# dronefreak/CABiNet

Hardware: AMD Instinct MI355X
Metric: 1024x1024 images/sec fwd+bwd (CABiNet-MobileNetV3-Large) (higher is better)
Workload: dtype f32; 1 GPU; BASELINE configs[2]: CABiNet-MobileNetV3-Large, 8x3x1024x1024 synthetic 8-class per GPU, fwd + 2x OhemCE + bwd + grad all-reduce + SGD step, HIP CAB/FFM kernels, fp32, random-init (model seed 0, gamma=0.5); per_gpu_batch=8, global_batch=8, n_classes=8, parallelism=dp1, miopen_find_mode=FAST

## Files before the change

cabinet_amd/_lib.py:

```python

from __future__ import annotations

import ctypes
import os
import threading

_PKG_DIR = os.path.dirname(os.path.abspath(__file__))
LIB_PATH = os.path.join(_PKG_DIR, "libcabinet_hip.so")
ABI_VERSION = 8

_c_float_p = ctypes.c_void_p
_INT, _FLT, _SZ, _PTR = ctypes.c_int, ctypes.c_float, ctypes.c_size_t, ctypes.c_void_p

SIGNATURES = {
    "cabinet_abi_version": (_INT, []),
    "cabinet_last_error": (ctypes.c_char_p, []),
    "cabinet_cab_attn_supported": (_INT, [_INT] * 2),
    "cabinet_cab_attn_precision_supported": (_INT, [_INT] * 3),
    "cabinet_cab_attn_fwd_workspace_bytes": (_SZ, [_INT] * 5),
    "cabinet_cab_attn_fwd": (_INT, [_PTR, _PTR, _PTR, _FLT, _INT, _INT, _INT, _INT, _INT, _PTR, _PTR, _PTR, _SZ, _PTR]),
    "cabinet_cab_attn_proj_supported": (_INT, [_INT] * 5),
    "cabinet_cab_attn_proj_fwd": (_INT, [_PTR] * 4 + [_FLT] + [_INT] * 5 + [_PTR] * 3 + [_PTR]),
    "cabinet_cab_attn_bwd_workspace_bytes": (_SZ, [_INT] * 4),
    "cabinet_cab_attn_bwd": (_INT, [_PTR] * 6 + [_FLT] + [_INT] * 4 + [_PTR] * 3 + [_PTR, _SZ, _PTR]),
    "cabinet_ffm_fwd_workspace_bytes": (_SZ, [_INT] * 7),
    "cabinet_ffm_fwd": (_INT, [_PTR] * 9 + [_INT] * 7 + [_INT, _FLT, _FLT] + [_PTR] * 6 + [_PTR, _SZ, _PTR]),
    "cabinet_ffm_bwd_workspace_bytes": (_SZ, [_INT] * 7),
    "cabinet_ffm_bwd": (_INT, [_PTR] * 13 + [_INT] * 7 + [_INT] + [_PTR] * 7 + [_PTR, _SZ, _PTR]),
    "cabinet_ffm_up_fwd_workspace_bytes": (_SZ, [_INT] * 9),
    "cabinet_ffm_up_fwd": (_INT, [_PTR] * 9 + [_INT] * 9 + [_INT, _FLT, _FLT, _INT] + [_PTR] * 6 + [_PTR, _SZ, _PTR]),
    "cabinet_ffm_up_bwd_workspace_bytes": (_SZ, [_INT] * 9),
    "cabinet_ffm_up_bwd": (_INT, [_PTR] * 13 + [_INT] * 9 + [_INT] + [_PTR] * 7 + [_PTR, _SZ, _PTR]),
    "cabinet_ohem_up_blocks": (_INT, [_INT] * 3),
    "cabinet_ohem_stats": (_INT, [_PTR, _PTR, _INT, _INT, _PTR, _PTR]),
    "cabinet_ohem_up_fwd": (_INT, [_PTR, _PTR] + [_INT] * 6 + [_FLT, _INT] + [_PTR] * 3 + [_PTR]),
    "cabinet_ohem_up_bwd_workspace_bytes": (_SZ, [_INT] * 6),
    "cabinet_ohem_up_bwd": (_INT, [_PTR] * 3 + [_INT] * 6 + [_FLT, _INT, _FLT] + [_PTR] + [_PTR, _SZ, _PTR]),
    "cabinet_ohem_up_pair_fwd": (_INT, [_PTR] * 3 + [_INT] * 6 + [_FLT, _INT] + [_PTR] * 3 + [_PTR]),
    "cabinet_ohem_up_pair_bwd_workspace_bytes": (_SZ, [_INT] * 6),
    "cabinet_ohem_up_pair_bwd": (_INT, [_PTR] * 4 + [_INT] * 6 + [_FLT, _INT, _FLT] + [_PTR] + [_PTR, _SZ, _PTR]),
    "cabinet_ohem_up_w_fwd": (_INT, [_PTR, _PTR] + [_INT] * 6 + [_FLT, _INT] + [_PTR] * 3 + [_PTR, _PTR]),
    "cabinet_ohem_up_w_bwd": (_INT, [_PTR] * 3 + [_INT] * 6 + [_FLT, _INT, _FLT] + [_PTR] + [_PTR, _SZ] + [_PTR, _PTR]),
    "cabinet_ohem_up_pair_w_fwd": (_INT, [_PTR] * 3 + [_INT] * 6 + [_FLT, _INT] + [_PTR] * 3 + [_PTR, _PTR, _PTR]),
    "cabinet_ohem_up_pair_w_bwd": (_INT, [_PTR] * 4 + [_INT] * 6 + [_FLT, _INT, _FLT] + [_PTR] + [_PTR, _SZ] + [_PTR, _PTR, _PTR]),
    "cabinet_ohem_select_workspace_bytes": (_SZ, [_INT] * 4),
    "cabinet_ohem_select": (_INT, [_PTR] * 3 + [_INT] * 5 + [_FLT] + [_INT] * 3 + [_PTR] * 3 + [_PTR, _SZ, _PTR]),
    "cabinet_ohem_up_w_bwd_sel": (_INT, [_PTR] * 3 + [_INT] * 6 + [_PTR, _INT, _FLT] + [_PTR] + [_PTR, _SZ] + [_PTR, _PTR]),
    "cabinet_ohem_up_pair_w_bwd_sel": (_INT, [_PTR] * 4 + [_INT] * 6 + [_PTR, _INT, _FLT] + [_PTR] + [_PTR, _SZ] + [_PTR, _PTR, _PTR]),
    "cabinet_cab_qkv_supported": (_INT, [_INT] * 7 + [_PTR]),
    "cabinet_cab_qkv_padded_bins": (_INT, [_INT, _PTR]),
    "cabinet_cab_qkv_fwd_workspace_bytes": (_SZ, [_INT] * 7 + [_PTR]),
    "cabinet_cab_qkv_fwd": (_INT, [_PTR] * 14 + [_INT] * 7 + [_PTR] + [_INT, _FLT, _FLT] + [_PTR] * 10
                            + [_PTR, _SZ, _PTR]),
    "cabinet_cab_qkv_bwd_workspace_bytes": (_SZ, [_INT] * 7 + [_PTR]),
    "cabinet_cab_qkv_bwd": (_INT, [_PTR] * 20 + [_INT] * 7 + [_PTR] + [_INT] + [_PTR] * 9 + [_PTR, _SZ, _PTR]),
    "cabinet_conv1x1_fwd_workspace_bytes": (_SZ, [_INT] * 2),
    "cabinet_conv1x1_fwd": (_INT, [_PTR] * 2 + [_INT] * 4 + [_PTR] + [_PTR, _SZ, _PTR]),
    "cabinet_conv1x1_bias_supported": (_INT, [_INT] * 4),
    "cabinet_conv1x1_bias_fwd": (_INT, [_PTR] * 3 + [_INT] * 4 + [_PTR] + [_PTR, _SZ, _PTR]),
    "cabinet_channel_sum": (_INT, [_PTR] + [_INT] * 3 + [_PTR] + [_PTR]),
    "cabinet_conv1x1_bwd_workspace_bytes": (_SZ, [_INT] * 4),
    "cabinet_conv1x1_bwd": (_INT, [_PTR] * 3 + [_INT] * 4 + [_PTR] * 2 + [_PTR, _SZ, _PTR]),
    "cabinet_bn_act_workspace_bytes": (_SZ, [_INT] * 3),
    "cabinet_bn_act_fwd": (_INT, [_PTR] * 6 + [_INT] * 5 + [_FLT, _FLT] + [_PTR] * 3 + [_PTR, _SZ, _PTR]),
    "cabinet_bn_act_bwd": (_INT, [_PTR] * 6 + [_INT] * 5 + [_PTR] * 3 + [_PTR, _SZ, _PTR]),
    "cabinet_bn_cls_supported": (_INT, [_INT] * 3),
    "cabinet_bn_cls_table_floats": (_INT, [_INT] * 2),
    "cabinet_bn_cls_fwd_workspace_bytes": (_SZ, [_INT] * 3),
    "cabinet_bn_cls_fwd": (_INT, [_PTR] * 8 + [_INT] * 6 + [_FLT, _FLT] + [_PTR] * 2 + [_PTR, _SZ, _PTR]),
    "cabinet_bn_cls_bwd_workspace_bytes": (_SZ, [_INT] * 4),
    "cabinet_bn_cls_bwd": (_INT, [_PTR] * 3 + [_INT] * 6 + [_PTR] * 5 + [_PTR, _SZ, _PTR]),
    "cabinet_gate_act_fwd": (_INT, [_PTR] * 2 + [_INT] * 4 + [_PTR] + [_PTR]),
    "cabinet_gate_act_bwd_workspace_bytes": (_SZ, [_INT] * 3),
    "cabinet_gate_act_bwd": (_INT, [_PTR] * 3 + [_INT] * 4 + [_PTR] * 2 + [_PTR, _SZ, _PTR]),
    "cabinet_bn_dwconv_fwd_workspace_bytes": (_SZ, [_INT] * 4),
    "cabinet_bn_dwconv_fwd": (_INT, [_PTR] * 6 + [_INT] * 8 + [_FLT, _FLT] + [_PTR] * 3 + [_PTR, _SZ, _PTR]),
    "cabinet_bn_dwconv_bwd_workspace_bytes": (_SZ, [_INT] * 6),
    "cabinet_bn_dwconv_bwd": (_INT, [_PTR] * 7 + [_INT] * 8 + [_PTR] * 4 + [_PTR, _SZ, _PTR]),
    "cabinet_stem_conv_fwd": (_INT, [_PTR] * 2 + [_INT] * 3 + [_PTR] + [_PTR]),
    "cabinet_stem_conv_wrw_workspace_bytes": (_SZ, [_INT] * 3),
    "cabinet_stem_conv_wrw": (_INT, [_PTR] * 2 + [_INT] * 3 + [_PTR] + [_PTR, _SZ, _PTR]),
    "cabinet_pwconv_supported": (_INT, [_INT] * 3),
    "cabinet_pwconv_fwd": (_INT, [_PTR] * 2 + [_INT] * 4 + [_PTR] + [_PTR]),
    "cabinet_pwconv_bwd_workspace_bytes": (_SZ, [_INT] * 4),
    "cabinet_pwconv_bwd": (_INT, [_PTR] * 3 + [_INT] * 4 + [_PTR] * 2 + [_PTR, _SZ, _PTR]),
    "cabinet_pwconv_wide_supported": (_INT, [_INT] * 3),
    "cabinet_pwconv_wide_wgrad_workspace_bytes": (_SZ, [_INT] * 4),
    "cabinet_pwconv_wide_wgrad": (_INT, [_PTR] * 2 + [_INT] * 4 + [_PTR] + [_PTR, _SZ, _PTR]),
    "cabinet_conv3x3s2_supported": (_INT, [_INT] * 2),
    "cabinet_conv3x3s2_wgrad_workspace_bytes": (_SZ, [_INT] * 5),
    "cabinet_conv3x3s2_wgrad": (_INT, [_PTR] * 2 + [_INT] * 5 + [_PTR] + [_PTR, _SZ, _PTR]),
    "cabinet_conv3x3s2_dgrad": (_INT, [_PTR] * 2 + [_INT] * 5 + [_PTR] + [_PTR]),
    "cabinet_bn_act_fwd_part": (_INT, [_PTR] * 7 + [_INT] * 6 + [_FLT, _FLT] + [_PTR] * 3 + [_PTR]),
    "cabinet_conv3x3_supported": (_INT, [_INT] * 3),
    "cabinet_conv3x3_tile_blocks": (_INT, [_INT] * 3),
    "cabinet_conv3x3_fwd_workspace_bytes": (_SZ, [_INT] * 6),
    "cabinet_conv3x3_fwd": (_INT, [_PTR] * 3 + [_INT] * 6 + [_PTR] * 2 + [_PTR, _SZ, _PTR]),
    "cabinet_conv3x3_bwd_workspace_bytes": (_SZ, [_INT] * 6),
    "cabinet_conv3x3_bwd": (_INT, [_PTR] * 4 + [_INT] * 6 + [_PTR] * 3 + [_PTR, _SZ, _PTR]),
    "cabinet_dwconv_supported": (_INT, [_INT] * 2),
    "cabinet_dwconv_fwd": (_INT, [_PTR] * 2 + [_INT] * 6 + [_PTR] + [_PTR]),
    "cabinet_dwconv_bwd_workspace_bytes": (_SZ, [_INT] * 6),
    "cabinet_dwconv_bwd": (_INT, [_PTR] * 3 + [_INT] * 6 + [_PTR] * 2 + [_PTR, _SZ, _PTR]),
    "cabinet_cab_local_supported": (_INT, [_INT] * 4),
    "cabinet_cab_local_fwd_workspace_bytes": (_SZ, [_INT] * 4),
    "cabinet_cab_local_bwd_workspace_bytes": (_SZ, [_INT] * 4),
    "cabinet_cab_local_fwd": (_INT, [_PTR] * 3 + [_PTR] * 5 + [_INT] * 5 + [_FLT, _FLT] + [_PTR] * 3 + [_PTR, _SZ, _PTR]),
    "cabinet_cab_local_bwd": (_INT, [_PTR] * 4 + [_PTR] * 3 + [_PTR] * 2 + [_INT] * 5 + [_PTR] * 3 + [_PTR] * 3 + [_PTR, _SZ, _PTR]),
    "cabinet_eval_chip_accum_supported": (_INT, [_INT] * 6),
    "cabinet_eval_chip_accum": (_INT, [_PTR] * 2 + [_INT] * 6 + [_PTR] + [_INT] * 4 + [_PTR] * 2 + [_PTR]),
    "cabinet_eval_scale_merge": (_INT, [_PTR] + [_INT] * 8 + [_PTR] + [_INT] * 2 + [_PTR]),
    "cabinet_eval_argmax_hist": (_INT, [_PTR] * 2 + [_INT] * 5 + [_PTR] * 2 + [_PTR]),
    "cabinet_se_act_bwd_workspace_bytes": (_SZ, [_INT] * 3),
    "cabinet_se_act_bwd_reduce": (_INT, [_PTR] * 8 + [_INT] * 4 + [_PTR] * 2 + [_PTR, _SZ, _PTR]),
    "cabinet_se_act_bwd_coef": (_INT, [_PTR] * 3 + [_INT] * 4 + [_PTR] * 4 + [_PTR]),
    "cabinet_se_act_bwd_dx": (_INT, [_PTR] * 9 + [_INT] * 4 + [_PTR] + [_PTR]),
}

_lock = threading.Lock()
_lib = None


def _preload_hip_runtime():
    import sys

    cands = []
    if "torch" in sys.modules:
        cands.append(os.path.join(os.path.dirname(sys.modules["torch"].__file__), "lib", "libamdhip64.so"))
    cands += ["libamdhip64.so.7", "/opt/rocm/lib/libamdhip64.so.7"]
    for c in cands:
        try:
            ctypes.CDLL(c, mode=ctypes.RTLD_GLOBAL)
            return c
        except OSError:
            continue
    raise RuntimeError("cabinet_amd: no HIP runtime (libamdhip64.so.7) could be loaded")


def load():
    global _lib
    if _lib is not None:
        return _lib
    with _lock:
        if _lib is not None:
            return _lib
        if not os.path.exists(LIB_PATH):
            raise RuntimeError(
                f"cabinet_amd: {LIB_PATH} is missing -- build it with `python -m cabinet_amd.build` "
                "(there is no non-HIP fallback for device tensors)")
        _preload_hip_runtime()
        lib = ctypes.CDLL(LIB_PATH)
        for name, (res, args) in SIGNATURES.items():
            try:
                fn = getattr(lib, name)
            except AttributeError as e:
                raise RuntimeError(f"cabinet_amd: {LIB_PATH} does not export {name}") from e
            fn.restype, fn.argtypes = res, args
        got = lib.cabinet_abi_version()
        if got != ABI_VERSION:
            raise RuntimeError(f"cabinet_amd: ABI version {got} != expected {ABI_VERSION}; rebuild the library")
        _lib = lib
    return _lib


def available() -> bool:
    return os.path.exists(LIB_PATH)


def check(rc: int, what: str):
    if rc != 0:
        msg = load().cabinet_last_error().decode("utf-8", "replace")
        raise RuntimeError(f"cabinet_amd: {what} failed (code {rc}): {msg}")
```

cabinet_amd/build.py:

```python

from __future__ import annotations

import argparse
import hashlib
import os
import shutil
import subprocess
import sys
from concurrent.futures import ThreadPoolExecutor

PKG_DIR = os.path.dirname(os.path.abspath(__file__))
CSRC = os.path.join(PKG_DIR, "csrc")
OBJ_DIR = os.path.join(PKG_DIR, "csrc", "build")
LIB_PATH = os.path.join(PKG_DIR, "libcabinet_hip.so")
ARCH = "gfx950"

SOURCES = ["capi.hip", "cab_attn_fwd.hip", "cab_attn_bf16.hip", "cab_attn_bwd.hip", "ffm.hip", "ffm_bwd_fused.hip", "ffm_bwd_adj.hip", "ffm_fwd_fused.hip", "gemm_bf16.hip", "ohem.hip", "cab_local.hip", "cab_local_tiled.hip", "cab_qkv.hip", "cab_qkv_fused.hip", "bn_act.hip", "dwconv.hip", "stem_conv.hip", "pwconv.hip", "pwconv_wide.hip", "conv3x3_s2.hip", "small_gemm.hip", "conv3x3_wino.hip", "bn_cls.hip", "eval_tail.hip"]
HEADERS = ["common.hpp", "cab_local.hpp", "cab_qkv.hpp", "blocks.hpp", "act.hpp", "bn_finalize.hpp", "slab_sum.hpp", os.path.join("..", "..", "include", "cabinet_hip.h")]


def _hipcc():
    for cand in (os.environ.get("HIPCC"), shutil.which("hipcc"), "/opt/rocm/bin/hipcc"):
        if cand and os.path.exists(cand):
            return cand
    raise RuntimeError("hipcc not found: cannot build libcabinet_hip.so")


def _digest(paths):
    h = hashlib.sha256()
    for p in paths:
        with open(p, "rb") as f:
            h.update(f.read())
    return h.hexdigest()


def source_digest():
    paths = [os.path.join(CSRC, s) for s in SOURCES] + [os.path.normpath(os.path.join(CSRC, h)) for h in HEADERS]
    return _digest(paths)


def is_fresh():
    stamp = LIB_PATH + ".stamp"
    if not (os.path.exists(LIB_PATH) and os.path.exists(stamp)):
        return False
    with open(stamp) as f:
        return f.read().strip() == _stamp()


def _stamp():
    return (source_digest() + " " + os.environ.get("CABINET_EXTRA_HIPCC_FLAGS", "").strip()).strip()


def build(force=False, save_temps=False, verbose=True):
    if not force and is_fresh():
        if verbose:
            print(f"[cabinet_amd.build] up to date: {LIB_PATH}")
        return LIB_PATH
    hipcc = _hipcc()
    os.makedirs(OBJ_DIR, exist_ok=True)
    flags = [f"--offload-arch={ARCH}", "-O3", "-fPIC", "-std=c++17", "-ffp-contract=off",
             "-Wall", "-Wno-unused-function"]
    if save_temps:
        flags.append("-save-temps=obj")
    flags += os.environ.get("CABINET_EXTRA_HIPCC_FLAGS", "").split()

    def compile_one(src):
        obj = os.path.join(OBJ_DIR, src.replace(".hip", ".o"))
        cmd = [hipcc, *flags, "-c", os.path.join(CSRC, src), "-o", obj]
        r = subprocess.run(cmd, capture_output=True, text=True)
        if r.returncode != 0:
            raise RuntimeError(f"hipcc failed for {src}:\n{r.stdout}\n{r.stderr}")
        if verbose and r.stderr.strip():
            print(r.stderr, file=sys.stderr)
        return obj

    with ThreadPoolExecutor(max_workers=min(len(SOURCES), os.cpu_count() or 4)) as ex:
        objs = list(ex.map(compile_one, SOURCES))
    link = [hipcc, f"--offload-arch={ARCH}", "-shared", "-fPIC", *objs, "-o", LIB_PATH,
            "-fno-rtlib-add-rpath", "-Wl,-soname,libcabinet_hip.so", "--hip-link"]
    r = subprocess.run(link, capture_output=True, text=True)
    if r.returncode != 0:
        raise RuntimeError(f"link failed:\n{r.stdout}\n{r.stderr}")
    with open(LIB_PATH + ".stamp", "w") as f:
        f.write(_stamp())
    if verbose:
        print(f"[cabinet_amd.build] built {LIB_PATH}")
    return LIB_PATH


if __name__ == "__main__":
    ap = argparse.ArgumentParser()
    ap.add_argument("--force", action="store_true")
    ap.add_argument("--save-temps", action="store_true")
    a = ap.parse_args()
    build(force=a.force, save_temps=a.save_temps)
```

cabinet_amd/csrc/act.hpp:

```cpp
#pragma once
#include <hip/hip_runtime.h>

namespace cabinet {

enum { ACT_NONE = 0, ACT_RELU = 1, ACT_HSWISH = 2 };

__device__ __forceinline__ float div6(float x) {
    const float c = 1.f / 6.f;
    const float q = x * c;
    return fmaf(fmaf(-6.f, q, x), c, q);
}

__device__ __forceinline__ float act_fwd(float u, int act) {
    if (act == ACT_RELU) return fmaxf(u, 0.f);
    if (act == ACT_HSWISH) return div6(u * fminf(fmaxf(u + 3.f, 0.f), 6.f));
    return u;
}
__device__ __forceinline__ float act_grad(float u, int act) {
    if (act == ACT_RELU) return u > 0.f ? 1.f : 0.f;
    if (act == ACT_HSWISH) {
        const float t = u + 3.f;
        const float inner = (t > 0.f && t < 6.f) ? div6(u) : 0.f;
        return div6(fminf(fmaxf(t, 0.f), 6.f)) + inner;
    }
    return 1.f;
}

struct BnFold {
    const float *mean, *invstd, *weight, *bias;
    int act;
};

size_t bn_act_workspace(int B, int C, int P);
hipError_t bn_stats_run(const float* x, float* running_mean, float* running_var, int B, int C, int P, int training,
                        float momentum, float eps, float* save_mean, float* save_invstd, void* ws, hipStream_t stream);
hipError_t bn_bwd_tail_run(const float* part, int nt, const float* dy, const float* x, const float* weight,
                           const float* bias, const float* save_mean, const float* save_invstd, int B, int C, int P,
                           int act, int training, float* dx, float* dweight, float* dbias, float* coef,
                           hipStream_t stream);

}
```

cabinet_amd/csrc/bn_act.hip:

```cpp
#include "act.hpp"
#include "bn_finalize.hpp"
#include "common.hpp"

namespace cabinet {


__device__ __forceinline__ int ba_load(const float* __restrict__ row, int P, int lo, f32x4 (&v)[BA_V]) {
    const int hi = min(lo + BA_CHUNK, P);
    if ((P & 3) == 0) {
#pragma unroll
        for (int i = 0; i < BA_V; ++i) {
            const int p = lo + (i * BA_T + threadIdx.x) * 4;
            v[i] = p < hi ? *reinterpret_cast<const f32x4*>(row + p) : f32x4{0.f, 0.f, 0.f, 0.f};
        }
    } else {
#pragma unroll
        for (int i = 0; i < BA_V; ++i)
#pragma unroll
            for (int e = 0; e < 4; ++e) {
                const int p = lo + (i * BA_T + threadIdx.x) * 4 + e;
                v[i][e] = p < hi ? row[p] : 0.f;
            }
    }
    return hi - lo;
// ... 215 lines not shown
    f32x4 vz[BA_V], vg[BA_V];
    ba_load(z + (size_t)row * P, P, ch * BA_CHUNK, vz);
    ba_load(dy + (size_t)row * P, P, ch * BA_CHUNK, vg);
    float s1 = 0.f, s2 = 0.f, s3 = 0.f;
#pragma unroll
    for (int i = 0; i < BA_V; ++i)
#pragma unroll
        for (int e = 0; e < 4; ++e) {
            const float xh = (vz[i][e] - mu) * inv;
            const float du = vg[i][e] * act_grad(fmaf(xh, gam, bet) * gt, act);
            s1 += du, s2 = fmaf(du, xh, s2);
            if (ba_valid(P, ch * BA_CHUNK, i, e)) s3 += xh;
        }
    s1 = block_sum_256(s1, red);
    s2 = block_sum_256(s2, red);
    s3 = block_sum_256(s3, red);
    if (threadIdx.x == 0) {
        part[(size_t)row * chunks + ch] = s1;
        part[((size_t)rows + row) * chunks + ch] = s2;
        part[((size_t)2 * rows + row) * chunks + ch] = s3;
    }
}

__global__ void se_bwd_gate_kernel(const float* __restrict__ part, int rows, int C, int chunks, const float* __restrict__ weight,
                                   const float* __restrict__ bias, const float* __restrict__ a2, float* __restrict__ sums,
                                   float* __restrict__ da2) {
    const int row = blockIdx.x * blockDim.x + threadIdx.x;
    if (row >= rows) return;
    float s[3];
#pragma unroll
    for (int k = 0; k < 3; ++k) {
        float t = 0.f;
        for (int j = 0; j < chunks; ++j) t += part[((size_t)k * rows + row) * chunks + j];
        sums[(size_t)k * rows + row] = s[k] = t;
    }
    const int c = row % C;
    const float dgate = weight[c] * s[1] + bias[c] * s[0], u = a2[row] + 3.f;
    da2[row] = (u > 0.f && u < 6.f) ? dgate / 6.f : 0.f;
}

__global__ void se_bwd_coef_kernel(const float* __restrict__ sums, const float* __restrict__ gate, const float* __restrict__ ds,
                                   int B, int C, int P, int training, float* __restrict__ dweight, float* __restrict__ dbias,
                                   float* __restrict__ coef, float* __restrict__ ds_p) {
    const int c = blockIdx.x * blockDim.x + threadIdx.x;
    if (c >= C) return;
    const int rows = B * C;
    float db = 0.f, dw = 0.f;
    for (int b = 0; b < B; ++b) {
        const int row = b * C + c;
        const float g = gate[row], d = ds[row], dp = d / (float)P;
        ds_p[row] = dp;
        db += g * sums[row] + d;
        dw += g * sums[rows + row] + dp * sums[2 * rows + row];
    }
    dbias[c] = db;
    dweight[c] = dw;
    const float n = (float)B * (float)P;
    coef[c] = training ? db / n : 0.f;
    coef[C + c] = training ? dw / n : 0.f;
}

__global__ __launch_bounds__(BA_T) void se_bwd_dx_kernel(const float* __restrict__ dy, const float* __restrict__ z,
                                                         const float* __restrict__ mean, const float* __restrict__ invstd,
                                                         const float* __restrict__ weight, const float* __restrict__ bias,
                                                         const float* __restrict__ gate, const float* __restrict__ ds_p,
                                                         const float* __restrict__ coef, int C, int P, int chunks, int act,
                                                         float* __restrict__ dz) {
    const int row = blockIdx.x / chunks, ch = blockIdx.x - row * chunks, c = row % C;
    const float mu = mean[c], inv = invstd[c], gam = weight[c], bet = bias[c], gt = gate[row], dp = ds_p[row];
    const float m1 = coef[c], m2 = coef[C + c], gi = gam * inv;
    f32x4 vz[BA_V], vg[BA_V];
    ba_load(z + (size_t)row * P, P, ch * BA_CHUNK, vz);
    ba_load(dy + (size_t)row * P, P, ch * BA_CHUNK, vg);
#pragma unroll
    for (int i = 0; i < BA_V; ++i)
#pragma unroll
        for (int e = 0; e < 4; ++e) {
            const float xh = (vz[i][e] - mu) * inv;
            const float du = vg[i][e] * act_grad(fmaf(xh, gam, bet) * gt, act);
            vg[i][e] = gi * (fmaf(gt, du, dp) - m1 - xh * m2);
        }
    ba_store(dz + (size_t)row * P, P, ch * BA_CHUNK, vg);
}

static int ba_chunks(int P) { return ceil_div(P, BA_CHUNK); }

size_t se_act_bwd_workspace(int B, int C, int P) { return align_up((size_t)3 * B * C * ba_chunks(P) * sizeof(float), 256); }

hipError_t se_act_bwd_reduce_run(const float* dy, const float* z, const float* mean, const float* invstd, const float* weight,
                                 const float* bias, const float* gate, const float* a2, int B, int C, int P, int act, float* sums,
                                 float* da2, void* ws, hipStream_t stream) {
    const int chunks = ba_chunks(P), rows = B * C;
    float* part = static_cast<float*>(ws);
    hipLaunchKernelGGL(se_bwd_reduce_kernel, dim3(rows * chunks), dim3(BA_T), 0, stream, dy, z, mean, invstd, weight, bias, gate,
                       rows, C, P, chunks, act, part);
    hipLaunchKernelGGL(se_bwd_gate_kernel, dim3(ceil_div(rows, 256)), dim3(256), 0, stream, part, rows, C, chunks, weight, bias, a2,
                       sums, da2);
    return hipGetLastError();
}

hipError_t se_act_bwd_coef_run(const float* sums, const float* gate, const float* ds, int B, int C, int P, int training,
                               float* dweight, float* dbias, float* coef, float* ds_p, hipStream_t stream) {
    hipLaunchKernelGGL(se_bwd_coef_kernel, dim3(ceil_div(C, 256)), dim3(256), 0, stream, sums, gate, ds, B, C, P, training, dweight,
                       dbias, coef, ds_p);
    return hipGetLastError();
}

hipError_t se_act_bwd_dx_run(const float* dy, const float* z, const float* mean, const float* invstd, const float* weight,
                             const float* bias, const float* gate, const float* ds_p, const float* coef, int B, int C, int P,
                             int act, float* dz, hipStream_t stream) {
    const int chunks = ba_chunks(P);
    hipLaunchKernelGGL(se_bwd_dx_kernel, dim3(B * C * chunks), dim3(BA_T), 0, stream, dy, z, mean, invstd, weight, bias, gate,
                       ds_p, coef, C, P, chunks, act, dz);
    return hipGetLastError();
}

size_t bn_act_workspace(int B, int C, int P) {
    return align_up((size_t)2 * C * B * ba_chunks(P) * sizeof(float), 256) + align_up((size_t)2 * C * sizeof(float), 256);
}

hipError_t bn_stats_run(const float* x, float* running_mean, float* running_var, int B, int C, int P, int training,
                        float momentum, float eps, float* save_mean, float* save_invstd, void* ws, hipStream_t stream) {
    const int chunks = ba_chunks(P), grid = B * C * chunks;
    float* part = static_cast<float*>(ws);
    if (training)
        hipLaunchKernelGGL(bn_act_stats_kernel, dim3(grid), dim3(BA_T), 0, stream, x, part, B, C, P, chunks);
    hipLaunchKernelGGL(bn_act_finalize_kernel, dim3(C), dim3(BA_T), 0, stream, part, B, C, P, chunks, 0, 0, training, momentum,
                       eps, running_mean, running_var, save_mean, save_invstd);
    return hipGetLastError();
}

hipError_t bn_act_fwd_part_run(const float* x, const float* conv_part, int H, int W, const float* weight, const float* bias,
                               float* running_mean, float* running_var, const float* residual, int B, int C, int act, int training,
                               float momentum, float eps, float* y, float* save_mean, float* save_invstd, hipStream_t stream) {
    const int P = H * W, chunks = ba_chunks(P), grid = B * C * chunks;
    hipLaunchKernelGGL(bn_act_finalize_kernel, dim3(C), dim3(BA_T), 0, stream, conv_part, B, C, P, chunks, H, W, training, momentum,
                       eps, running_mean, running_var, save_mean, save_invstd);
    hipLaunchKernelGGL(bn_act_apply_kernel, dim3(grid), dim3(BA_T), 0, stream, x, save_mean, save_invstd, weight, bias,
                       residual, C, P, chunks, act, y);
    return hipGetLastError();
}

hipError_t bn_act_fwd_run(const float* x, const float* weight, const float* bias, float* running_mean,
                          float* running_var, const float* residual, int B, int C, int P, int act, int training,
                          float momentum, float eps, float* y, float* save_mean, float* save_invstd, void* ws,
                          hipStream_t stream) {
    const int chunks = ba_chunks(P), grid = B * C * chunks;
    (void)bn_stats_run(x, running_mean, running_var, B, C, P, training, momentum, eps, save_mean, save_invstd, ws, stream);
    hipLaunchKernelGGL(bn_act_apply_kernel, dim3(grid), dim3(BA_T), 0, stream, x, save_mean, save_invstd, weight, bias,
                       residual, C, P, chunks, act, y);
    return hipGetLastError();
}

hipError_t bn_bwd_tail_run(const float* part, int nt, const float* dy, const float* x, const float* weight,
                           const float* bias, const float* save_mean, const float* save_invstd, int B, int C, int P,
                           int act, int training, float* dx, float* dweight, float* dbias, float* coef,
                           hipStream_t stream) {
    const int chunks = ba_chunks(P), grid = B * C * chunks;
    hipLaunchKernelGGL(bn_act_bwd_finalize_kernel, dim3(C), dim3(BA_T), 0, stream, part, nt, C, (double)B * (double)P,
                       training, dweight, dbias, coef);
    hipLaunchKernelGGL(bn_act_bwd_dx_kernel, dim3(grid), dim3(BA_T), 0, stream, dy, x, save_mean, save_invstd, weight,
                       bias, coef, C, P, chunks, act, dx);
    return hipGetLastError();
}

hipError_t bn_act_bwd_run(const float* dy, const float* x, const float* weight, const float* bias,
                          const float* save_mean, const float* save_invstd, int B, int C, int P, int act, int training,
                          float* dx, float* dweight, float* dbias, void* ws, hipStream_t stream) {
    const int chunks = ba_chunks(P), grid = B * C * chunks, nt = B * chunks;
    float* part = static_cast<float*>(ws);
    float* coef = reinterpret_cast<float*>(static_cast<char*>(ws) + align_up((size_t)2 * C * nt * sizeof(float), 256));
    hipLaunchKernelGGL(bn_act_bwd_reduce_kernel, dim3(grid), dim3(BA_T), 0, stream, dy, x, save_mean, save_invstd, weight,
                       bias, B, C, P, chunks, act, part);
    return bn_bwd_tail_run(part, nt, dy, x, weight, bias, save_mean, save_invstd, B, C, P, act, training, dx, dweight,
                           dbias, coef, stream);
}

size_t gate_act_workspace(int rows, int P) { return align_up((size_t)rows * ba_chunks(P) * sizeof(float), 256); }

hipError_t gate_act_fwd_run(const float* x, const float* gate, int rows, int P, int act, float* y, hipStream_t stream) {
    const int chunks = ba_chunks(P);
    hipLaunchKernelGGL(gate_act_fwd_kernel, dim3(rows * chunks), dim3(BA_T), 0, stream, x, gate, P, chunks, act, y);
    return hipGetLastError();
}

hipError_t gate_act_bwd_run(const float* dy, const float* x, const float* gate, int rows, int P, int act, float* dx,
                            float* dgate, void* ws, hipStream_t stream) {
    const int chunks = ba_chunks(P);
    float* part = static_cast<float*>(ws);
    hipLaunchKernelGGL(gate_act_bwd_kernel, dim3(rows * chunks), dim3(BA_T), 0, stream, dy, x, gate, P, chunks, act, dx,
                       part);
    hipLaunchKernelGGL(gate_act_dgate_kernel, dim3(ceil_div(rows, 256)), dim3(256), 0, stream, part, rows, chunks, dgate);
    return hipGetLastError();
}

}
```

cabinet_amd/csrc/capi.hip:

```cpp
#include "../../include/cabinet_hip.h"

#include <stdarg.h>
#include <stdint.h>
#include <stdio.h>

#include "blocks.hpp"
#include "cab_local.hpp"
#include "cab_qkv.hpp"
#include "common.hpp"

namespace cabinet {
int attn_fwd_kvsplit(int B, int n);
bool attn_shape_supported(int Kc, int Vc);
hipError_t attn_fwd_dispatch(const float* q, const float* k, const float* v, float scale, int B, int Kc,
                             int Vc, int n, float* ctx, float* lse, float* part_ctx, float* part_lse,
                             int kvsplit, hipStream_t stream);
bool attn_fwd_proj_supported(int B, int Kc, int Vc, int Co, int n);
hipError_t attn_fwd_proj_dispatch(const float* q, const float* k, const float* v, const float* w_out, float scale, int B, int Kc,
                                  int Vc, int Co, int n, float* ctx, float* glob, float* lse, hipStream_t stream);
bool attn_bf16_supported(int Kc, int Vc);
size_t attn_bf16_pack_bytes(int B, int Kc, int Vc, int n, int precision);
hipError_t attn_fwd_bf16_dispatch(const float* q, const float* k, const float* v, float scale, int B, int Kc, int Vc, int n,
                                  float* ctx, float* lse, float* part_ctx, float* part_lse, int kvsplit, void* pack, int precision,
                                  hipStream_t stream);
size_t attn_bwd_workspace(int B, int Kc, int Vc, int n);
hipError_t attn_bwd_dispatch(const float* dctx, const float* q, const float* k, const float* v,
                             const float* ctx, const float* lse, float scale, int B, int Kc, int Vc, int n,
                             float* dq, float* dk, float* dv, void* ws, hipStream_t stream);
struct FfmShape {
    int B, Cs, Cc, Co, Cm, H, W;
};
size_t ffm_fwd_workspace(const FfmShape& s);
size_t ffm_bwd_workspace(const FfmShape& s);
hipError_t ffm_fwd_run(const FfmShape& s, const float* fsp, const float* fcp, const float* w_blk,
                       const float* bn_w, const float* bn_b, float* run_mean, float* run_var,
                       const float* w1, const float* w2, int training, float momentum, float eps, float* out,
                       float* z, float* save_mean, float* save_invstd, float* pooled, float* gate, void* ws,
                       hipStream_t stream);
size_t ffm_up_fwd_workspace(const FfmShape& s, int Hl, int Wl);
size_t ffm_up_bwd_workspace(const FfmShape& s, int Hl, int Wl);
hipError_t ffm_up_fwd_run(const FfmShape& s, int Hl, int Wl, const float* fsp, const float* low,
                          const float* w_blk, const float* bn_w, const float* bn_b, float* run_mean,
                          float* run_var, const float* w1, const float* w2, int training, float momentum,
                          float eps, float* out, float* z, float* save_mean, float* save_invstd, float* pooled,
                          float* gate, void* ws, int precision, hipStream_t stream);
hipError_t ffm_up_bwd_run(const FfmShape& s, int Hl, int Wl, const float* dout, const float* fsp,
                          const float* low, const float* w_blk, const float* bn_w, const float* bn_b,
                          const float* w1, const float* w2, const float* z, const float* save_mean,
                          const float* save_invstd, const float* pooled, const float* gate, int training,
                          float* dfsp, float* dlow, float* dw_blk, float* dbn_w, float* dbn_b, float* dw1,
                          float* dw2, void* ws, hipStream_t stream);
hipError_t ffm_bwd_run(const FfmShape& s, const float* dout, const float* fsp, const float* fcp,
                       const float* w_blk, const float* bn_w, const float* bn_b, const float* w1,
                       const float* w2, const float* z, const float* save_mean, const float* save_invstd,
                       const float* pooled, const float* gate, int training, float* dfsp, float* dfcp,
                       float* dw_blk, float* dbn_w, float* dbn_b, float* dw1, float* dw2, void* ws,
                       hipStream_t stream);
size_t bn_act_workspace(int B, int C, int P);
hipError_t bn_act_fwd_run(const float* x, const float* weight, const float* bias, float* running_mean,
                          float* running_var, const float* residual, int B, int C, int P, int act, int training,
                          float momentum, float eps, float* y, float* save_mean, float* save_invstd, void* ws,
                          hipStream_t stream);
hipError_t bn_act_bwd_run(const float* dy, const float* x, const float* weight, const float* bias,
                          const float* save_mean, const float* save_invstd, int B, int C, int P, int act, int training,
                          float* dx, float* dweight, float* dbias, void* ws, hipStream_t stream);
hipError_t bn_act_fwd_part_run(const float* x, const float* conv_part, int H, int W, const float* weight, const float* bias,
                               float* running_mean, float* running_var, const float* residual, int B, int C, int act, int training,
                               float momentum, float eps, float* y, float* save_mean, float* save_invstd, hipStream_t stream);
size_t se_act_bwd_workspace(int B, int C, int P);
hipError_t se_act_bwd_reduce_run(const float* dy, const float* z, const float* mean, const float* invstd, const float* weight,
                                 const float* bias, const float* gate, const float* a2, int B, int C, int P, int act, float* sums,
                                 float* da2, void* ws, hipStream_t stream);
hipError_t se_act_bwd_coef_run(const float* sums, const float* gate, const float* ds, int B, int C, int P, int training,
                               float* dweight, float* dbias, float* coef, float* ds_p, hipStream_t stream);
hipError_t se_act_bwd_dx_run(const float* dy, const float* z, const float* mean, const float* invstd, const float* weight,
                             const float* bias, const float* gate, const float* ds_p, const float* coef, int B, int C, int P,
                             int act, float* dz, hipStream_t stream);
size_t gate_act_workspace(int rows, int P);
hipError_t gate_act_fwd_run(const float* x, const float* gate, int rows, int P, int act, float* y, hipStream_t stream);
hipError_t gate_act_bwd_run(const float* dy, const float* x, const float* gate, int rows, int P, int act, float* dx,
                            float* dgate, void* ws, hipStream_t stream);
bool bn_cls_supported(int C, int K, int P);
int bn_cls_table_floats(int C, int K);
size_t bn_cls_fwd_workspace(int B, int C, int P);
size_t bn_cls_bwd_workspace(int B, int C, int K, int P);
hipError_t bn_cls_fwd_run(const float* z, const float* conv_part, const float* bn_w, const float* bn_b, float* run_mean, float* run_var,
                          const float* w_cls, const float* bias, int B, int C, int K, int H, int W, int training, float momentum,
                          float eps, float* y, float* tab, void* ws, hipStream_t stream);
hipError_t bn_cls_bwd_run(const float* dy, const float* z, const float* tab, int B, int C, int K, int H, int W, int training, float* dz,
                          float* dbn_w, float* dbn_b, float* dw_cls, float* dbias, void* ws, hipStream_t stream);
bool dwconv_supported(int K, int S);
size_t dwconv_bwd_workspace(int B, int C, int H, int W, int K);
hipError_t dwconv_fwd_run(const float* x, const float* w, int B, int C, int H, int W, int K, int S, float* y,
                          hipStream_t stream);
hipError_t dwconv_bwd_run(const float* dy, const float* x, const float* w, int B, int C, int H, int W, int K, int S,
                          float* dx, float* dw, void* ws, hipStream_t stream);
size_t bn_dwconv_fwd_workspace(int B, int C, int H, int W);
size_t bn_dwconv_bwd_workspace(int B, int C, int H, int W, int K);
hipError_t bn_dwconv_fwd_run(const float* z, const float* bn_w, const float* bn_b, float* run_mean, float* run_var,
                             const float* w, int B, int C, int H, int W, int K, int S, int act, int training,
                             float momentum, float eps, float* y, float* save_mean, float* save_invstd, void* ws,
                             hipStream_t stream);
hipError_t bn_dwconv_bwd_run(const float* dy, const float* z, const float* bn_w, const float* bn_b,
                             const float* save_mean, const float* save_invstd, const float* w, int B, int C, int H,
                             int W, int K, int S, int act, int training, float* dz, float* dbn_w, float* dbn_b,
                             float* dw, void* ws, hipStream_t stream);
size_t stem_conv_wrw_workspace(int B, int H, int W);
hipError_t stem_conv_fwd_run(const float* x, const float* w, int B, int H, int W, float* y, hipStream_t stream);
hipError_t stem_conv_wrw_run(const float* dy, const float* x, int B, int H, int W, float* dw, void* ws,
                             hipStream_t stream);
bool pwconv_wide_supported(int Ci, int Co, int P);
size_t pwconv_wide_wgrad_workspace(int B, int Ci, int Co, int P);
hipError_t pwconv_wide_wgrad_run(const float* dy, const float* x, int B, int Ci, int Co, int P, float* dw, void* ws,
                                 hipStream_t stream);
bool conv3x3s2_supported(int Ci, int Co);
long long conv3x3s2_wgrad_slabs(int B, int Ci, int H, int W);
size_t conv3x3s2_wgrad_workspace(int B, int Ci, int H, int W);
hipError_t conv3x3s2_wgrad_run(const float* dy, const float* x, int B, int Ci, int H, int W, float* dw, void* ws,
                               hipStream_t stream);
long long conv3x3s2_dgrad_workgroups(int B, int H, int W);
hipError_t conv3x3s2_dgrad_run(const float* dy, const float* w, int B, int H, int W, float* dx, hipStream_t stream);
bool pwconv_supported(int Ci, int Co, int P);
size_t pwconv_bwd_workspace(int B, int Ci, int Co, int P);
hipError_t pwconv_fwd_run(const float* x, const float* w, int B, int Ci, int Co, int P, float* y, hipStream_t stream);
hipError_t pwconv_bwd_run(const float* dy, const float* x, const float* w, int B, int Ci, int Co, int P, float* dx,
                          float* dw, void* ws, hipStream_t stream);
int ohem_blocks(int B, int H, int W);
hipError_t ohem_up_fwd_run(int nh, const float* const* low, const long long* labels, int B, int C, int Hl, int Wl, int H, int W,
                           float thresh, int ignore_lb, float* const* loss_px, float* const* blk_sum, int* const* blk_cnt,
                           const float* const* class_weight, hipStream_t stream);
hipError_t ohem_stats_run(const float* blk_sum, const int* blk_cnt, int nheads, int nblk, double* stats, hipStream_t stream);
size_t ohem_up_bwd_workspace(int B, int C, int H, int Wl);
bool ohem_up_supported(int C, int Wl, int W);
hipError_t ohem_up_bwd_run(int nh, const float* const* low, const long long* labels, const float* const* loss_px, int B, int C,
                           int Hl, int Wl, int H, int W, float thresh, int ignore_lb, float coef, float* dlow, void* ws,
                           const float* const* cw, const double* dsel, hipStream_t stream);
size_t ohem_select_workspace(int nheads);
hipError_t ohem_select_run(int nheads, const float* const* loss_px, const long long* labels, const double* stats, long long P, int C,
                           float thresh, const int* n_min, int ignore_lb, const float* const* cw, double* sel, void* ws,
                           hipStream_t stream);
struct WinoShape {
    int B, C0, C1, K, H, W;
};
bool conv3x3_supported(int C0, int C1, int K);
bool conv3x3_shape_ok(const WinoShape& s);
int conv3x3_tile_blocks(int B, int H, int W);
size_t conv3x3_fwd_workspace(const WinoShape& s);
size_t conv3x3_bwd_workspace(const WinoShape& s);
hipError_t conv3x3_fwd_run(const WinoShape& s, const float* x0, const float* x1, const float* w, float* y, float* stat_part, void* ws,
                           hipStream_t stream);
hipError_t conv3x3_bwd_run(const WinoShape& s, const float* dy, const float* x0, const float* x1, const float* w, float* dx0,
                           float* dx1, float* dw, void* ws, hipStream_t stream);
int eval_chip_threads(int C, int wl, int cw, int nsrc);
hipError_t eval_chip_accum_run(const float* a, const float* b, int N, int C, int hl, int wl, int ch, int cw, float* dst, int FH,
                               int FW, int y0, int x0, const float* rcp_y, const float* rcp_x, hipStream_t stream);
hipError_t eval_scale_merge_run(const float* prob, int N, int C, int FH, int FW, int hst, int hed, int wst, int wed, float* total,
                                int H, int W, hipStream_t stream);
hipError_t eval_argmax_hist_run(const float* total, const long long* labels, int N, int C, int H, int W, int ignore_lb, long long* hist,
                                unsigned char* pred, hipStream_t stream);
}

static thread_local char g_err[512] = "";

static int fail(int code, const char* fmt, ...) {
    va_list ap;
    va_start(ap, fmt);
    vsnprintf(g_err, sizeof(g_err), fmt, ap);
    va_end(ap);
    return code;
}

template <typename... P>
static bool aligned16(P... p) {
    return ((reinterpret_cast<uintptr_t>(p) | ...) & 15) == 0;
}
#define CABINET_REQUIRE_ALIGNED(what, ...)                                                                            \
    if (!aligned16(__VA_ARGS__))                                                                                      \
    return fail(CABINET_ERR_INVALID_ARG, what ": tensor pointers must be 16-byte aligned (128-bit loads / stores)")

static int hip_status(hipError_t e, const char* what) {
    if (e == hipSuccess) return CABINET_OK;
    return fail(CABINET_ERR_HIP, "%s: %s", what, hipGetErrorString(e));
}

extern "C" {

int cabinet_abi_version(void) { return CABINET_ABI_VERSION; }
const char* cabinet_last_error(void) { return g_err; }

static int check_attn_shape(int B, int Kc, int Vc, int n) {
    if (B <= 0 || Kc <= 0 || Vc <= 0 || n <= 0)
        return fail(CABINET_ERR_INVALID_ARG, "cab_attn: non-positive dimension B=%d Kc=%d Vc=%d n=%d", B, Kc,
                    Vc, n);
    if (!cabinet::attn_shape_supported(Kc, Vc))
        return fail(CABINET_ERR_UNSUPPORTED,
                    "cab_attn: (Kc=%d, Vc=%d) has no gfx950 instantiation; built: (128,128) (256,128) (64,64)",
                    Kc, Vc);
    if (B > 65535) return fail(CABINET_ERR_UNSUPPORTED, "cab_attn: B=%d exceeds grid.z", B);
    return CABINET_OK;
}

int cabinet_cab_attn_supported(int Kc, int Vc) { return cabinet::attn_shape_supported(Kc, Vc) ? 1 : 0; }

int cabinet_cab_attn_precision_supported(int Kc, int Vc, int precision) {
    if (precision == CABINET_PREC_FP32) return cabinet_cab_attn_supported(Kc, Vc);
    if (precision == CABINET_PREC_BF16X3 || precision == CABINET_PREC_BF16X6) return cabinet::attn_bf16_supported(Kc, Vc) ? 1 : 0;
    return 0;
}

static size_t attn_fwd_split_bytes(int B, int Vc, int n, int split) {
    if (split == 1) return 0;
    return align_up((size_t)split * B * Vc * n * sizeof(float), 256) + align_up((size_t)split * B * n * sizeof(float), 256);
}

size_t cabinet_cab_attn_fwd_workspace_bytes(int B, int Kc, int Vc, int n, int precision) {
    if (B <= 0 || Kc <= 0 || Vc <= 0 || n <= 0 || !cabinet_cab_attn_precision_supported(Kc, Vc, precision)) return 0;
    const size_t pack = precision == CABINET_PREC_FP32 ? 0 : cabinet::attn_bf16_pack_bytes(B, Kc, Vc, n, precision);
    return attn_fwd_split_bytes(B, Vc, n, cabinet::attn_fwd_kvsplit(B, n)) + pack;
}

int cabinet_cab_attn_fwd(const float* q, const float* k, const float* v, float scale, int B, int Kc, int Vc,
                         int n, int precision, float* ctx, float* lse, void* workspace, size_t workspace_bytes,
                         cabinet_stream_t stream) {
    if (int rc = check_attn_shape(B, Kc, Vc, n)) return rc;
    if (!cabinet_cab_attn_precision_supported(Kc, Vc, precision))
        return fail(CABINET_ERR_UNSUPPORTED, "cab_attn_fwd: precision %d is not built for (Kc=%d, Vc=%d)", precision, Kc, Vc);
    if (!q || !k || !v || !ctx || !lse) return fail(CABINET_ERR_INVALID_ARG, "cab_attn_fwd: null tensor pointer");
    CABINET_REQUIRE_ALIGNED("cab_attn_fwd", q, k, v, ctx, lse);
    const size_t need = cabinet_cab_attn_fwd_workspace_bytes(B, Kc, Vc, n, precision);
    if (need && (!workspace || workspace_bytes < need))
        return fail(CABINET_ERR_WORKSPACE, "cab_attn_fwd: workspace %zu < %zu bytes", workspace_bytes, need);
    const int split = cabinet::attn_fwd_kvsplit(B, n);
    float* part_ctx = static_cast<float*>(workspace);
    float* part_lse = split > 1 ? reinterpret_cast<float*>(static_cast<char*>(workspace) +
                                                           align_up((size_t)split * B * Vc * n * sizeof(float), 256))
                                : nullptr;
    if (precision != CABINET_PREC_FP32) {
        void* pack = static_cast<char*>(workspace) + attn_fwd_split_bytes(B, Vc, n, split);
        return hip_status(cabinet::attn_fwd_bf16_dispatch(q, k, v, scale, B, Kc, Vc, n, ctx, lse, part_ctx, part_lse, split, pack,
                                                          precision, static_cast<hipStream_t>(stream)),
                          "cab_attn_fwd (split bf16) launch");
    }
    return hip_status(cabinet::attn_fwd_dispatch(q, k, v, scale, B, Kc, Vc, n, ctx, lse, part_ctx, part_lse,
                                                 split, static_cast<hipStream_t>(stream)),
                      "cab_attn_fwd launch");
}

int cabinet_cab_attn_proj_supported(int B, int Kc, int Vc, int Co, int n) {
    return cabinet::attn_fwd_proj_supported(B, Kc, Vc, Co, n) ? 1 : 0;
}

int cabinet_cab_attn_proj_fwd(const float* q, const float* k, const float* v, const float* w_out, float scale, int B, int Kc,
                              int Vc, int Co, int n, float* ctx, float* glob, float* lse, cabinet_stream_t stream) {
    if (int rc = check_attn_shape(B, Kc, Vc, n)) return rc;
    if (Co <= 0) return fail(CABINET_ERR_INVALID_ARG, "cab_attn_proj_fwd: non-positive Co=%d", Co);
    if (!cabinet::attn_fwd_proj_supported(B, Kc, Vc, Co, n))
        return fail(CABINET_ERR_UNSUPPORTED,
                    "cab_attn_proj_fwd: (B=%d, Kc=%d, Vc=%d, Co=%d, n=%d) is outside the fused form (see "
                    "cabinet_cab_attn_proj_supported); use cabinet_cab_attn_fwd + cabinet_conv1x1_fwd",
                    B, Kc, Vc, Co, n);
    if (!q || !k || !v || !w_out || !glob || !lse) return fail(CABINET_ERR_INVALID_ARG, "cab_attn_proj_fwd: null tensor pointer");
    CABINET_REQUIRE_ALIGNED("cab_attn_proj_fwd", q, k, v, w_out, ctx, glob, lse);
    return hip_status(cabinet::attn_fwd_proj_dispatch(q, k, v, w_out, scale, B, Kc, Vc, Co, n, ctx, glob, lse,
// ... 703 lines not shown
                       int stride, float* dx, float* dw, void* workspace, size_t workspace_bytes,
                       cabinet_stream_t stream) {
    if (int rc = check_dwconv(B, C, H, W, K, stride, "dwconv_bwd")) return rc;
    if (!dy || !x || !weight || !dx || !dw) return fail(CABINET_ERR_INVALID_ARG, "dwconv_bwd: null tensor pointer");
    const size_t need = cabinet::dwconv_bwd_workspace(B, C, H, W, K);
    if (!workspace || workspace_bytes < need)
        return fail(CABINET_ERR_WORKSPACE, "dwconv_bwd: workspace %zu < %zu bytes", workspace_bytes, need);
    return hip_status(cabinet::dwconv_bwd_run(dy, x, weight, B, C, H, W, K, stride, dx, dw, workspace,
                                              static_cast<hipStream_t>(stream)),
                      "dwconv_bwd launch");
}

int cabinet_gate_act_fwd(const float* x, const float* gate, int B, int C, int P, int act, float* y,
                         cabinet_stream_t stream) {
    if (int rc = check_bn_act(B, C, P, act, "gate_act_fwd")) return rc;
    if (!x || !gate || !y) return fail(CABINET_ERR_INVALID_ARG, "gate_act_fwd: null tensor pointer");
    return hip_status(cabinet::gate_act_fwd_run(x, gate, B * C, P, act, y, static_cast<hipStream_t>(stream)),
                      "gate_act_fwd launch");
}

size_t cabinet_gate_act_bwd_workspace_bytes(int B, int C, int P) {
    return B > 0 && C > 0 && P > 0 ? cabinet::gate_act_workspace(B * C, P) : 0;
}

int cabinet_gate_act_bwd(const float* dy, const float* x, const float* gate, int B, int C, int P, int act, float* dx,
                         float* dgate, void* workspace, size_t workspace_bytes, cabinet_stream_t stream) {
    if (int rc = check_bn_act(B, C, P, act, "gate_act_bwd")) return rc;
    if (!dy || !x || !gate || !dx || !dgate) return fail(CABINET_ERR_INVALID_ARG, "gate_act_bwd: null tensor pointer");
    const size_t need = cabinet::gate_act_workspace(B * C, P);
    if (!workspace || workspace_bytes < need)
        return fail(CABINET_ERR_WORKSPACE, "gate_act_bwd: workspace %zu < %zu bytes", workspace_bytes, need);
    return hip_status(cabinet::gate_act_bwd_run(dy, x, gate, B * C, P, act, dx, dgate, workspace,
                                                static_cast<hipStream_t>(stream)),
                      "gate_act_bwd launch");
}

size_t cabinet_se_act_bwd_workspace_bytes(int B, int C, int P) {
    return B > 0 && C > 0 && P > 0 ? cabinet::se_act_bwd_workspace(B, C, P) : 0;
}

int cabinet_se_act_bwd_reduce(const float* dy, const float* z, const float* mean, const float* invstd, const float* bn_weight,
                              const float* bn_bias, const float* gate, const float* a2, int B, int C, int P, int act, float* sums,
                              float* da2, void* workspace, size_t workspace_bytes, cabinet_stream_t stream) {
    if (int rc = check_bn_act(B, C, P, act, "se_act_bwd_reduce")) return rc;
    if (!dy || !z || !mean || !invstd || !bn_weight || !bn_bias || !gate || !a2 || !sums || !da2)
        return fail(CABINET_ERR_INVALID_ARG, "se_act_bwd_reduce: null tensor pointer");
    CABINET_REQUIRE_ALIGNED("se_act_bwd_reduce", dy, z);
    const size_t need = cabinet::se_act_bwd_workspace(B, C, P);
    if (!workspace || workspace_bytes < need)
        return fail(CABINET_ERR_WORKSPACE, "se_act_bwd_reduce: workspace %zu < %zu bytes", workspace_bytes, need);
    return hip_status(cabinet::se_act_bwd_reduce_run(dy, z, mean, invstd, bn_weight, bn_bias, gate, a2, B, C, P, act, sums, da2,
                                                     workspace, static_cast<hipStream_t>(stream)),
                      "se_act_bwd_reduce launch");
}

int cabinet_se_act_bwd_coef(const float* sums, const float* gate, const float* ds, int B, int C, int P, int training,
                            float* dbn_weight, float* dbn_bias, float* coef, float* ds_over_p, cabinet_stream_t stream) {
    if (B <= 0 || C <= 0 || P <= 0) return fail(CABINET_ERR_INVALID_ARG, "se_act_bwd_coef: non-positive dimension");
    if (!sums || !gate || !ds || !dbn_weight || !dbn_bias || !coef || !ds_over_p)
        return fail(CABINET_ERR_INVALID_ARG, "se_act_bwd_coef: null tensor pointer");
    return hip_status(cabinet::se_act_bwd_coef_run(sums, gate, ds, B, C, P, training, dbn_weight, dbn_bias, coef, ds_over_p,
                                                   static_cast<hipStream_t>(stream)),
                      "se_act_bwd_coef launch");
}

int cabinet_se_act_bwd_dx(const float* dy, const float* z, const float* mean, const float* invstd, const float* bn_weight,
                          const float* bn_bias, const float* gate, const float* ds_over_p, const float* coef, int B, int C, int P,
                          int act, float* dz, cabinet_stream_t stream) {
    if (int rc = check_bn_act(B, C, P, act, "se_act_bwd_dx")) return rc;
    if (!dy || !z || !mean || !invstd || !bn_weight || !bn_bias || !gate || !ds_over_p || !coef || !dz)
        return fail(CABINET_ERR_INVALID_ARG, "se_act_bwd_dx: null tensor pointer");
    CABINET_REQUIRE_ALIGNED("se_act_bwd_dx", dy, z, dz);
    return hip_status(cabinet::se_act_bwd_dx_run(dy, z, mean, invstd, bn_weight, bn_bias, gate, ds_over_p, coef, B, C, P, act, dz,
                                                 static_cast<hipStream_t>(stream)),
                      "se_act_bwd_dx launch");
}

size_t cabinet_bn_dwconv_fwd_workspace_bytes(int B, int C, int H, int W) {
    return B > 0 && C > 0 && H > 0 && W > 0 ? cabinet::bn_dwconv_fwd_workspace(B, C, H, W) : 0;
}

int cabinet_bn_dwconv_fwd(const float* z, const float* bn_weight, const float* bn_bias, float* running_mean,
                          float* running_var, const float* conv_weight, int B, int C, int H, int W, int K, int stride,
                          int act, int training, float momentum, float eps, float* y, float* save_mean,
                          float* save_invstd, void* workspace, size_t workspace_bytes, cabinet_stream_t stream) {
    if (int rc = check_dwconv(B, C, H, W, K, stride, "bn_dwconv_fwd")) return rc;
    if (int rc = check_bn_act(B, C, H * W, act, "bn_dwconv_fwd")) return rc;
    if (!z || !bn_weight || !bn_bias || !running_mean || !running_var || !conv_weight || !y || !save_mean || !save_invstd)
        return fail(CABINET_ERR_INVALID_ARG, "bn_dwconv_fwd: null tensor pointer");
    const size_t need = cabinet::bn_dwconv_fwd_workspace(B, C, H, W);
    if (!workspace || workspace_bytes < need)
        return fail(CABINET_ERR_WORKSPACE, "bn_dwconv_fwd: workspace %zu < %zu bytes", workspace_bytes, need);
    return hip_status(cabinet::bn_dwconv_fwd_run(z, bn_weight, bn_bias, running_mean, running_var, conv_weight, B, C, H, W,
                                                 K, stride, act, training, momentum, eps, y, save_mean, save_invstd,
                                                 workspace, static_cast<hipStream_t>(stream)),
                      "bn_dwconv_fwd launch");
}

size_t cabinet_bn_dwconv_bwd_workspace_bytes(int B, int C, int H, int W, int K, int stride) {
    if (B <= 0 || C <= 0 || H <= 0 || W <= 0 || !cabinet::dwconv_supported(K, stride)) return 0;
    return cabinet::bn_dwconv_bwd_workspace(B, C, H, W, K);
}

int cabinet_bn_dwconv_bwd(const float* dy, const float* z, const float* bn_weight, const float* bn_bias,
                          const float* save_mean, const float* save_invstd, const float* conv_weight, int B, int C,
                          int H, int W, int K, int stride, int act, int training, float* dz, float* dbn_weight,
                          float* dbn_bias, float* dconv_weight, void* workspace, size_t workspace_bytes,
                          cabinet_stream_t stream) {
    if (int rc = check_dwconv(B, C, H, W, K, stride, "bn_dwconv_bwd")) return rc;
    if (int rc = check_bn_act(B, C, H * W, act, "bn_dwconv_bwd")) return rc;
    if (!dy || !z || !bn_weight || !bn_bias || !save_mean || !save_invstd || !conv_weight || !dz || !dbn_weight ||
        !dbn_bias || !dconv_weight)
        return fail(CABINET_ERR_INVALID_ARG, "bn_dwconv_bwd: null tensor pointer");
    const size_t need = cabinet::bn_dwconv_bwd_workspace(B, C, H, W, K);
    if (!workspace || workspace_bytes < need)
        return fail(CABINET_ERR_WORKSPACE, "bn_dwconv_bwd: workspace %zu < %zu bytes", workspace_bytes, need);
    return hip_status(cabinet::bn_dwconv_bwd_run(dy, z, bn_weight, bn_bias, save_mean, save_invstd, conv_weight, B, C, H,
                                                 W, K, stride, act, training, dz, dbn_weight, dbn_bias, dconv_weight,
                                                 workspace, static_cast<hipStream_t>(stream)),
                      "bn_dwconv_bwd launch");
}

static int check_stem(int B, int H, int W, const char* who) {
    if (B <= 0 || H <= 0 || W <= 0) return fail(CABINET_ERR_INVALID_ARG, "%s: non-positive dimension", who);
    if ((long long)B * ((H + 1) / 2) > 2147483647LL / 4) return fail(CABINET_ERR_UNSUPPORTED, "%s: grid too large", who);
    return CABINET_OK;
}

int cabinet_stem_conv_fwd(const float* x, const float* weight, int B, int H, int W, float* y, cabinet_stream_t stream) {
    if (int rc = check_stem(B, H, W, "stem_conv_fwd")) return rc;
    if (!x || !weight || !y) return fail(CABINET_ERR_INVALID_ARG, "stem_conv_fwd: null tensor pointer");
    return hip_status(cabinet::stem_conv_fwd_run(x, weight, B, H, W, y, static_cast<hipStream_t>(stream)),
                      "stem_conv_fwd launch");
}

size_t cabinet_stem_conv_wrw_workspace_bytes(int B, int H, int W) {
    return B > 0 && H > 0 && W > 0 ? cabinet::stem_conv_wrw_workspace(B, H, W) : 0;
}

int cabinet_stem_conv_wrw(const float* dy, const float* x, int B, int H, int W, float* dw, void* workspace,
                          size_t workspace_bytes, cabinet_stream_t stream) {
    if (int rc = check_stem(B, H, W, "stem_conv_wrw")) return rc;
    if (!dy || !x || !dw) return fail(CABINET_ERR_INVALID_ARG, "stem_conv_wrw: null tensor pointer");
    const size_t need = cabinet::stem_conv_wrw_workspace(B, H, W);
    if (!workspace || workspace_bytes < need)
        return fail(CABINET_ERR_WORKSPACE, "stem_conv_wrw: workspace %zu < %zu bytes", workspace_bytes, need);
    return hip_status(cabinet::stem_conv_wrw_run(dy, x, B, H, W, dw, workspace, static_cast<hipStream_t>(stream)),
                      "stem_conv_wrw launch");
}

static int check_pwconv(int B, int Ci, int Co, int P, const char* who) {
    if (B <= 0 || Ci <= 0 || Co <= 0 || P <= 0) return fail(CABINET_ERR_INVALID_ARG, "%s: non-positive dimension", who);
    if (!cabinet::pwconv_supported(Ci, Co, P))
        return fail(CABINET_ERR_UNSUPPORTED, "%s: Ci=%d, Co=%d (multiples of 8, <= 120, block product <= 8)", who, Ci, Co);
    return CABINET_OK;
}

int cabinet_pwconv_supported(int Ci, int Co, int P) {
    return Ci > 0 && Co > 0 && P > 0 && cabinet::pwconv_supported(Ci, Co, P) ? 1 : 0;
}

int cabinet_pwconv_fwd(const float* x, const float* w, int B, int Ci, int Co, int P, float* y, cabinet_stream_t stream) {
    if (int rc = check_pwconv(B, Ci, Co, P, "pwconv_fwd")) return rc;
    if (!x || !w || !y) return fail(CABINET_ERR_INVALID_ARG, "pwconv_fwd: null tensor pointer");
    return hip_status(cabinet::pwconv_fwd_run(x, w, B, Ci, Co, P, y, static_cast<hipStream_t>(stream)),
                      "pwconv_fwd launch");
}

size_t cabinet_pwconv_bwd_workspace_bytes(int B, int Ci, int Co, int P) {
    if (B <= 0 || Ci <= 0 || Co <= 0 || P <= 0 || !cabinet::pwconv_supported(Ci, Co, P)) return 0;
    return cabinet::pwconv_bwd_workspace(B, Ci, Co, P);
}

int cabinet_pwconv_bwd(const float* dy, const float* x, const float* w, int B, int Ci, int Co, int P, float* dx,
                       float* dw, void* workspace, size_t workspace_bytes, cabinet_stream_t stream) {
    if (int rc = check_pwconv(B, Ci, Co, P, "pwconv_bwd")) return rc;
    if (!dy || !x || !w) return fail(CABINET_ERR_INVALID_ARG, "pwconv_bwd: null tensor pointer");
    const size_t need = cabinet::pwconv_bwd_workspace(B, Ci, Co, P);
    if (dw && (!workspace || workspace_bytes < need))
        return fail(CABINET_ERR_WORKSPACE, "pwconv_bwd: workspace %zu < %zu bytes", workspace_bytes, need);
    return hip_status(cabinet::pwconv_bwd_run(dy, x, w, B, Ci, Co, P, dx, dw, workspace, static_cast<hipStream_t>(stream)),
                      "pwconv_bwd launch");
}

int cabinet_pwconv_wide_supported(int Ci, int Co, int P) {
    return Ci > 0 && Co > 0 && P > 0 && cabinet::pwconv_wide_supported(Ci, Co, P) ? 1 : 0;
}

size_t cabinet_pwconv_wide_wgrad_workspace_bytes(int B, int Ci, int Co, int P) {
    if (B <= 0 || Ci <= 0 || Co <= 0 || P <= 0 || !cabinet::pwconv_wide_supported(Ci, Co, P)) return 0;
    if ((long long)B * ((P + 63) / 64) > (1ll << 30)) return 0;
    return cabinet::pwconv_wide_wgrad_workspace(B, Ci, Co, P);
}

int cabinet_pwconv_wide_wgrad(const float* dy, const float* x, int B, int Ci, int Co, int P, float* dw, void* workspace,
                              size_t workspace_bytes, cabinet_stream_t stream) {
    if (B <= 0 || Ci <= 0 || Co <= 0 || P <= 0)
        return fail(CABINET_ERR_INVALID_ARG, "pwconv_wide_wgrad: non-positive dimension");
    if ((long long)B * ((P + 63) / 64) > (1ll << 30))
        return fail(CABINET_ERR_UNSUPPORTED, "pwconv_wide_wgrad: B=%d, P=%d: more than 2^30 pixel chunks", B, P);
    if (!cabinet::pwconv_wide_supported(Ci, Co, P))
        return fail(CABINET_ERR_UNSUPPORTED, "pwconv_wide_wgrad: Ci=%d, Co=%d, P=%d (multiples of 8, <= 4096, P <= 2^21, max(Ci, Co) * P <= 2^28)",
                    Ci, Co, P);
    if (!dy || !x || !dw) return fail(CABINET_ERR_INVALID_ARG, "pwconv_wide_wgrad: null tensor pointer");
    const size_t need = cabinet::pwconv_wide_wgrad_workspace(B, Ci, Co, P);
    if (!workspace || workspace_bytes < need)
        return fail(CABINET_ERR_WORKSPACE, "pwconv_wide_wgrad: workspace %zu < %zu bytes", workspace_bytes, need);
    return hip_status(cabinet::pwconv_wide_wgrad_run(dy, x, B, Ci, Co, P, dw, workspace, static_cast<hipStream_t>(stream)),
                      "pwconv_wide_wgrad launch");
}

static bool conv3x3s2_size_ok(int B, int Ci, int H, int W) {
    return cabinet::conv3x3s2_wgrad_slabs(B, Ci, H, W) <= (1ll << 30);
}

int cabinet_conv3x3s2_supported(int Ci, int Co) { return cabinet::conv3x3s2_supported(Ci, Co) ? 1 : 0; }

size_t cabinet_conv3x3s2_wgrad_workspace_bytes(int B, int Ci, int Co, int H, int W) {
    if (B <= 0 || H <= 0 || W <= 0 || !cabinet::conv3x3s2_supported(Ci, Co) || !conv3x3s2_size_ok(B, Ci, H, W)) return 0;
    return cabinet::conv3x3s2_wgrad_workspace(B, Ci, H, W);
}

int cabinet_conv3x3s2_wgrad(const float* dy, const float* x, int B, int Ci, int Co, int H, int W, float* dw, void* workspace,
                            size_t workspace_bytes, cabinet_stream_t stream) {
    if (B <= 0 || Ci <= 0 || Co <= 0 || H <= 0 || W <= 0)
        return fail(CABINET_ERR_INVALID_ARG, "conv3x3s2_wgrad: non-positive dimension");
    if (!cabinet::conv3x3s2_supported(Ci, Co))
        return fail(CABINET_ERR_UNSUPPORTED, "conv3x3s2_wgrad: Ci=%d, Co=%d ((64, 64) and (3, 16) are compiled)", Ci, Co);
    if (!conv3x3s2_size_ok(B, Ci, H, W))
        return fail(CABINET_ERR_UNSUPPORTED, "conv3x3s2_wgrad: B=%d, H=%d, W=%d: grid too large", B, H, W);
    if (!dy || !x || !dw) return fail(CABINET_ERR_INVALID_ARG, "conv3x3s2_wgrad: null tensor pointer");
    const size_t need = cabinet::conv3x3s2_wgrad_workspace(B, Ci, H, W);
    if (!workspace || workspace_bytes < need)
        return fail(CABINET_ERR_WORKSPACE, "conv3x3s2_wgrad: workspace %zu < %zu bytes", workspace_bytes, need);
    return hip_status(cabinet::conv3x3s2_wgrad_run(dy, x, B, Ci, H, W, dw, workspace, static_cast<hipStream_t>(stream)),
                      "conv3x3s2_wgrad launch");
}

int cabinet_conv3x3s2_dgrad(const float* dy, const float* w, int B, int Ci, int Co, int H, int W, float* dx,
                            cabinet_stream_t stream) {
    if (B <= 0 || Ci <= 0 || Co <= 0 || H <= 0 || W <= 0)
        return fail(CABINET_ERR_INVALID_ARG, "conv3x3s2_dgrad: non-positive dimension");
    if (Ci != 64 || Co != 64)
        return fail(CABINET_ERR_UNSUPPORTED, "conv3x3s2_dgrad: Ci=%d, Co=%d ((64, 64) is compiled)", Ci, Co);
    if (cabinet::conv3x3s2_dgrad_workgroups(B, H, W) > (1ll << 30))
        return fail(CABINET_ERR_UNSUPPORTED, "conv3x3s2_dgrad: B=%d, H=%d, W=%d: grid too large", B, H, W);
    if (!dy || !w || !dx) return fail(CABINET_ERR_INVALID_ARG, "conv3x3s2_dgrad: null tensor pointer");
    if ((reinterpret_cast<size_t>(dx) & 7) != 0)
        return fail(CABINET_ERR_INVALID_ARG, "conv3x3s2_dgrad: dx must be 8-byte aligned");
    return hip_status(cabinet::conv3x3s2_dgrad_run(dy, w, B, H, W, dx, static_cast<hipStream_t>(stream)), "conv3x3s2_dgrad launch");
}

static int check_conv3x3(const cabinet::WinoShape& s, const char* who) {
    if (s.B <= 0 || s.C0 <= 0 || s.C1 < 0 || s.K <= 0 || s.H <= 0 || s.W <= 0)
        return fail(CABINET_ERR_INVALID_ARG, "%s: non-positive dimension", who);
    if (!cabinet::conv3x3_shape_ok(s))
        return fail(CABINET_ERR_UNSUPPORTED,
                    "%s: C0=%d C1=%d Co=%d H=%d W=%d (C0, C1 multiples of 16; Co, C0+C1 multiples of 64; C0 %% 64 == 0 when C1 > 0; "
                    "one image's tensors < 1 GiB)", who, s.C0, s.C1, s.K, s.H, s.W);
    return CABINET_OK;
}

int cabinet_conv3x3_supported(int C0, int C1, int Co) { return cabinet::conv3x3_supported(C0, C1, Co) ? 1 : 0; }

int cabinet_conv3x3_tile_blocks(int B, int H, int W) {
    return B > 0 && H > 0 && W > 0 ? cabinet::conv3x3_tile_blocks(B, H, W) : 0;
}

size_t cabinet_conv3x3_fwd_workspace_bytes(int B, int C0, int C1, int Co, int H, int W) {
    const cabinet::WinoShape s{B, C0, C1, Co, H, W};
    return B > 0 && H > 0 && W > 0 && cabinet::conv3x3_shape_ok(s) ? cabinet::conv3x3_fwd_workspace(s) : 0;
}

int cabinet_conv3x3_fwd(const float* x0, const float* x1, const float* w, int B, int C0, int C1, int Co, int H, int W, float* y,
                        float* bn_part, void* workspace, size_t workspace_bytes, cabinet_stream_t stream) {
    const cabinet::WinoShape s{B, C0, C1, Co, H, W};
    if (int rc = check_conv3x3(s, "conv3x3_fwd")) return rc;
    if (!x0 || !w || !y || (C1 > 0 && !x1)) return fail(CABINET_ERR_INVALID_ARG, "conv3x3_fwd: null tensor pointer");
    CABINET_REQUIRE_ALIGNED("conv3x3_fwd", x0, x1, w, y, bn_part);
    const size_t need = cabinet::conv3x3_fwd_workspace(s);
    if (!workspace || workspace_bytes < need)
        return fail(CABINET_ERR_WORKSPACE, "conv3x3_fwd: workspace %zu < %zu bytes", workspace_bytes, need);
    return hip_status(cabinet::conv3x3_fwd_run(s, x0, C1 > 0 ? x1 : nullptr, w, y, bn_part, workspace, static_cast<hipStream_t>(stream)),
                      "conv3x3_fwd launch");
}

size_t cabinet_conv3x3_bwd_workspace_bytes(int B, int C0, int C1, int Co, int H, int W) {
    const cabinet::WinoShape s{B, C0, C1, Co, H, W};
    return B > 0 && H > 0 && W > 0 && cabinet::conv3x3_shape_ok(s) ? cabinet::conv3x3_bwd_workspace(s) : 0;
}

int cabinet_conv3x3_bwd(const float* dy, const float* x0, const float* x1, const float* w, int B, int C0, int C1, int Co, int H,
                        int W, float* dx0, float* dx1, float* dw, void* workspace, size_t workspace_bytes, cabinet_stream_t stream) {
    const cabinet::WinoShape s{B, C0, C1, Co, H, W};
    if (int rc = check_conv3x3(s, "conv3x3_bwd")) return rc;
    if (!dy || !w || (dw && (!x0 || (C1 > 0 && !x1))) || (dx0 && C1 > 0 && !dx1))
        return fail(CABINET_ERR_INVALID_ARG, "conv3x3_bwd: null tensor pointer");
    CABINET_REQUIRE_ALIGNED("conv3x3_bwd", dy, x0, x1, w, dx0, dx1, dw);
    const size_t need = cabinet::conv3x3_bwd_workspace(s);
    if (!workspace || workspace_bytes < need)
        return fail(CABINET_ERR_WORKSPACE, "conv3x3_bwd: workspace %zu < %zu bytes", workspace_bytes, need);
    return hip_status(cabinet::conv3x3_bwd_run(s, dy, x0, C1 > 0 ? x1 : nullptr, w, dx0, C1 > 0 ? dx1 : nullptr, dw, workspace,
                                               static_cast<hipStream_t>(stream)),
                      "conv3x3_bwd launch");
}

int cabinet_eval_chip_accum_supported(int C, int hl, int wl, int ch, int cw, int flip) {
    if (C < 1 || C > 32 || hl < 1 || wl < 1 || ch < 1 || cw < 1 || ch > 65535) return 0;
    return cabinet::eval_chip_threads(C, wl, cw, flip ? 2 : 1) > 0 ? 1 : 0;
}

int cabinet_eval_chip_accum(const float* a, const float* b, int N, int C, int hl, int wl, int ch, int cw, float* dst, int FH, int FW,
                            int y0, int x0, const float* rcp_y, const float* rcp_x, cabinet_stream_t stream) {
    if (N <= 0 || C <= 0 || hl <= 0 || wl <= 0 || ch <= 0 || cw <= 0 || FH <= 0 || FW <= 0)
        return fail(CABINET_ERR_INVALID_ARG, "eval_chip_accum: non-positive dimension");
    if (!a || !dst) return fail(CABINET_ERR_INVALID_ARG, "eval_chip_accum: null tensor pointer");
    if (y0 < 0 || x0 < 0 || y0 > FH - ch || x0 > FW - cw)
        return fail(CABINET_ERR_INVALID_ARG, "eval_chip_accum: window (%d,%d)+(%d,%d) leaves the %dx%d destination", y0, x0, ch, cw, FH, FW);
    if (C > 32) return fail(CABINET_ERR_UNSUPPORTED, "eval_chip_accum: C=%d classes (max 32)", C);
    if (N > 65535 || ch > 65535) return fail(CABINET_ERR_UNSUPPORTED, "eval_chip_accum: N or chip height exceeds grid limits");
    if (!cabinet_eval_chip_accum_supported(C, hl, wl, ch, cw, b != nullptr))
        return fail(CABINET_ERR_UNSUPPORTED, "eval_chip_accum: C=%d x resize ratio %d/%d exceeds the LDS row buffers", C, wl, cw);
    return hip_status(cabinet::eval_chip_accum_run(a, b, N, C, hl, wl, ch, cw, dst, FH, FW, y0, x0, rcp_y, rcp_x,
                                                   static_cast<hipStream_t>(stream)),
                      "eval_chip_accum launch");
}

int cabinet_eval_scale_merge(const float* prob, int N, int C, int FH, int FW, int hst, int hed, int wst, int wed, float* total, int H,
                             int W, cabinet_stream_t stream) {
    if (N <= 0 || C <= 0 || FH <= 0 || FW <= 0 || H <= 0 || W <= 0)
        return fail(CABINET_ERR_INVALID_ARG, "eval_scale_merge: non-positive dimension");
    if (!prob || !total) return fail(CABINET_ERR_INVALID_ARG, "eval_scale_merge: null tensor pointer");
    if (hst < 0 || wst < 0 || hed <= hst || wed <= wst || hed > FH || wed > FW)
        return fail(CABINET_ERR_INVALID_ARG, "eval_scale_merge: crop [%d:%d, %d:%d] leaves the %dx%d source", hst, hed, wst, wed, FH, FW);
    if ((long long)N * C > 65535 || H > 65535) return fail(CABINET_ERR_UNSUPPORTED, "eval_scale_merge: N*C or H exceeds grid limits");
// ... 18 lines not shown
```

cabinet_amd/csrc/dwconv.hip:

```cpp
#include "act.hpp"
#include "common.hpp"

namespace cabinet {

constexpr int DW_T = 256;
constexpr int DW_OUT = 1024;

struct DwShape {
    int B, C, H, W, Ho, Wo;
};

static int dw_tile_w(int w) { return w > 32 ? 64 : w > 16 ? 32 : w > 8 ? 16 : 8; }

template <int K, int S>
__global__ __launch_bounds__(DW_T) void dwconv_fwd_kernel(const float* __restrict__ x, const float* __restrict__ wgt,
                                                           DwShape s, int TW, int tiles_x, int tiles_y, BnFold f,
                                                           float* __restrict__ y) {
    constexpr int PAD = K / 2;
    extern __shared__ __attribute__((aligned(16))) float smem[];
    const int TH = DW_OUT / TW;
    const int tile = blockIdx.x % (tiles_x * tiles_y), plane = blockIdx.x / (tiles_x * tiles_y);
    const int c = plane % s.C;
    const int oy0 = (tile / tiles_x) * TH, ox0 = (tile % tiles_x) * TW;
    const int in_h = (TH - 1) * S + K, in_w = (TW - 1) * S + K;
// ... 225 lines not shown
                for (int kx = 0; kx < K; ++kx) {
                    if (((px + PAD - kx) & 1) != 0) continue;
                    const int bb = (px + PAD - kx) / 2 - OLO;
                    acc[px] = fmaf(w[ky][kx], g[a][bb], acc[px]);
                    pw[ky * K + kx] = fmaf(xv[px], g[a][bb], pw[ky * K + kx]);
                }
        }
#pragma unroll
        for (int px = 0; px < 2; ++px) {
            const int xx = x0 + 2 * tm + px;
            if (yy < s.H && xx < s.W) dxp[(size_t)yy * s.W + xx] = acc[px];
            const float du = acc[px] * dact[px];
            s1 += du, s2 = fmaf(du, xh[px], s2);
        }
    }
    if (f.mean) {
        s1 = block_sum_256(s1, red4);
        s2 = block_sum_256(s2, red4);
        if (threadIdx.x == 0) {
            const int nt = s.B * ntile;
            bnpart[(size_t)c * nt + b * ntile + tile] = s1;
            bnpart[((size_t)s.C + c) * nt + b * ntile + tile] = s2;
        }
    }
    dw_reduce_partials<KK>(pw, red, part + ((size_t)c * (s.B * ntile) + (size_t)b * ntile + tile) * KK);
}

__global__ __launch_bounds__(256) void dwconv_dw_finalize_kernel(const float* __restrict__ part, int nparts, int KK,
                                                                  float* __restrict__ dw) {
    __shared__ double dred[4];
    const int c = blockIdx.x / KK, tap = blockIdx.x - c * KK;
    double t = 0.0;
    for (int i = threadIdx.x; i < nparts; i += 256) t += (double)part[((size_t)c * nparts + i) * KK + tap];
#pragma unroll
    for (int o = 32; o >= 1; o >>= 1) t += __shfl_xor(t, o, 64);
    if ((threadIdx.x & 63) == 0) dred[threadIdx.x >> 6] = t;
    __syncthreads();
    if (threadIdx.x == 0) dw[blockIdx.x] = (float)((dred[0] + dred[1]) + (dred[2] + dred[3]));
}

bool dwconv_supported(int K, int S) { return (K == 3 || K == 5) && (S == 1 || S == 2); }

static void out_size(int H, int W, int K, int S, int& Ho, int& Wo) {
    Ho = (H + 2 * (K / 2) - K) / S + 1;
    Wo = (W + 2 * (K / 2) - K) / S + 1;
}

size_t dwconv_bwd_workspace(int B, int C, int H, int W, int K) {
    const int TW = dw_tile_w(W), TH = DW_OUT / TW;
    return align_up((size_t)C * B * ceil_div(W, TW) * ceil_div(H, TH) * K * K * sizeof(float), 256);
}

static int bwd_tiles(int H, int W) {
    const int TW = dw_tile_w(W), TH = DW_OUT / TW;
    return ceil_div(W, TW) * ceil_div(H, TH);
}

template <int K, int S>
static hipError_t fwd_launch(const float* x, const float* w, const DwShape& s, const BnFold& f, float* y,
                             hipStream_t stream) {
    const int TW = dw_tile_w(s.Wo), TH = DW_OUT / TW;
    const int tiles_x = ceil_div(s.Wo, TW), tiles_y = ceil_div(s.Ho, TH);
    const size_t lds = (size_t)((TH - 1) * S + K) * ((TW - 1) * S + K) * sizeof(float);
    hipLaunchKernelGGL((dwconv_fwd_kernel<K, S>), dim3((unsigned)((size_t)s.B * s.C * tiles_x * tiles_y)), dim3(DW_T), lds,
                       stream, x, w, s, TW, tiles_x, tiles_y, f, y);
    return hipGetLastError();
}

template <int K, int S>
static hipError_t bwd_launch(const float* dy, const float* x, const float* w, const DwShape& s, const BnFold& f,
                             float* dx, float* dw, float* part, float* bnpart, hipStream_t stream) {
    const int TW = dw_tile_w(s.W), TH = DW_OUT / TW;
    const int tiles_x = ceil_div(s.W, TW), tiles_y = ceil_div(s.H, TH);
    const size_t tile_floats = S == 1 ? (size_t)(TH + K - 1) * (TW + K - 1) : (size_t)(TH / 2 + 2) * (TW / 2 + 2);
    const size_t lds = (tile_floats + (size_t)K * K * (DW_T + 8)) * sizeof(float);
    const dim3 grid((unsigned)((size_t)s.B * s.C * tiles_x * tiles_y));
    if (S == 1)
        hipLaunchKernelGGL((dwconv_bwd_s1_kernel<K>), grid, dim3(DW_T), lds, stream, dy, x, w, s, TW, tiles_x, tiles_y, f,
                           dx, part, bnpart);
    else
        hipLaunchKernelGGL((dwconv_bwd_s2_kernel<K>), grid, dim3(DW_T), lds, stream, dy, x, w, s, TW, tiles_x, tiles_y, f,
                           dx, part, bnpart);
    hipLaunchKernelGGL(dwconv_dw_finalize_kernel, dim3(s.C * K * K), dim3(256), 0, stream, part, s.B * tiles_x * tiles_y,
                       K * K, dw);
    return hipGetLastError();
}

static hipError_t fwd_dispatch(const float* x, const float* w, const DwShape& s, int K, int S, const BnFold& f, float* y,
                               hipStream_t stream) {
    if (K == 3 && S == 1) return fwd_launch<3, 1>(x, w, s, f, y, stream);
    if (K == 3 && S == 2) return fwd_launch<3, 2>(x, w, s, f, y, stream);
    if (K == 5 && S == 1) return fwd_launch<5, 1>(x, w, s, f, y, stream);
    return fwd_launch<5, 2>(x, w, s, f, y, stream);
}

static hipError_t bwd_dispatch(const float* dy, const float* x, const float* w, const DwShape& s, int K, int S,
                               const BnFold& f, float* dx, float* dw, float* part, float* bnpart, hipStream_t stream) {
    if (K == 3 && S == 1) return bwd_launch<3, 1>(dy, x, w, s, f, dx, dw, part, bnpart, stream);
    if (K == 3 && S == 2) return bwd_launch<3, 2>(dy, x, w, s, f, dx, dw, part, bnpart, stream);
    if (K == 5 && S == 1) return bwd_launch<5, 1>(dy, x, w, s, f, dx, dw, part, bnpart, stream);
    return bwd_launch<5, 2>(dy, x, w, s, f, dx, dw, part, bnpart, stream);
}

hipError_t dwconv_fwd_run(const float* x, const float* w, int B, int C, int H, int W, int K, int S, float* y,
                          hipStream_t stream) {
    DwShape s{B, C, H, W, 0, 0};
    out_size(H, W, K, S, s.Ho, s.Wo);
    return fwd_dispatch(x, w, s, K, S, BnFold{nullptr, nullptr, nullptr, nullptr, 0}, y, stream);
}

hipError_t dwconv_bwd_run(const float* dy, const float* x, const float* w, int B, int C, int H, int W, int K, int S,
                          float* dx, float* dw, void* ws, hipStream_t stream) {
    DwShape s{B, C, H, W, 0, 0};
    out_size(H, W, K, S, s.Ho, s.Wo);
    return bwd_dispatch(dy, x, w, s, K, S, BnFold{nullptr, nullptr, nullptr, nullptr, 0}, dx, dw, static_cast<float*>(ws),
                        nullptr, stream);
}

struct BnDwWs {
    size_t bn, part, bnpart, coef, da, total;
};
static BnDwWs bn_dw_layout(int B, int C, int H, int W, int K) {
    BnDwWs w{};
    size_t off = 0;
    auto take = [&](size_t bytes) {
        const size_t o = off;
        off += align_up(bytes, 256);
        return o;
    };
    const int nt = B * bwd_tiles(H, W);
    w.bn = take(bn_act_workspace(B, C, H * W));
    w.part = take((size_t)C * nt * K * K * sizeof(float));
    w.bnpart = take((size_t)2 * C * nt * sizeof(float));
    w.coef = take((size_t)2 * C * sizeof(float));
    w.da = take((size_t)B * C * H * W * sizeof(float));
    w.total = off;
    return w;
}
size_t bn_dwconv_fwd_workspace(int B, int C, int H, int W) { return bn_act_workspace(B, C, H * W); }
size_t bn_dwconv_bwd_workspace(int B, int C, int H, int W, int K) { return bn_dw_layout(B, C, H, W, K).total; }

hipError_t bn_dwconv_fwd_run(const float* z, const float* bn_w, const float* bn_b, float* run_mean, float* run_var,
                             const float* w, int B, int C, int H, int W, int K, int S, int act, int training,
                             float momentum, float eps, float* y, float* save_mean, float* save_invstd, void* ws,
                             hipStream_t stream) {
    hipError_t e = bn_stats_run(z, run_mean, run_var, B, C, H * W, training, momentum, eps, save_mean, save_invstd, ws,
                                stream);
    if (e != hipSuccess) return e;
    DwShape s{B, C, H, W, 0, 0};
    out_size(H, W, K, S, s.Ho, s.Wo);
    return fwd_dispatch(z, w, s, K, S, BnFold{save_mean, save_invstd, bn_w, bn_b, act}, y, stream);
}

hipError_t bn_dwconv_bwd_run(const float* dy, const float* z, const float* bn_w, const float* bn_b,
                             const float* save_mean, const float* save_invstd, const float* w, int B, int C, int H,
                             int W, int K, int S, int act, int training, float* dz, float* dbn_w, float* dbn_b,
                             float* dw, void* ws, hipStream_t stream) {
    const BnDwWs L = bn_dw_layout(B, C, H, W, K);
    char* base = static_cast<char*>(ws);
    auto at = [&](size_t o) { return reinterpret_cast<float*>(base + o); };
    DwShape s{B, C, H, W, 0, 0};
    out_size(H, W, K, S, s.Ho, s.Wo);
    hipError_t e = bwd_dispatch(dy, z, w, s, K, S, BnFold{save_mean, save_invstd, bn_w, bn_b, act}, at(L.da), dw,
                                at(L.part), at(L.bnpart), stream);
    if (e != hipSuccess) return e;
    return bn_bwd_tail_run(at(L.bnpart), B * bwd_tiles(H, W), at(L.da), z, bn_w, bn_b, save_mean, save_invstd, B, C,
                           H * W, act, training, dz, dbn_w, dbn_b, at(L.coef), stream);
}

}
```

cabinet_amd/csrc/pwconv.hip:

```cpp
#include "common.hpp"

namespace cabinet {

constexpr int PW_MAXB = 4;

template <int MB>
__global__ __launch_bounds__(64) void pw_stream_kernel(const float* __restrict__ a, int sm, int sk, int M, int K,
                                                        const float* __restrict__ x, int P, int nblocks,
                                                        int blocks_per_img, float* __restrict__ y) {
    extern __shared__ __attribute__((aligned(16))) float al[];
    const int lane = threadIdx.x, li = lane & 31, h = lane >> 5, ld = K + 1;
    for (int i0 = 0; i0 < 32 * MB * K; i0 += 64 * 8) {
        float v[8];
#pragma unroll
        for (int j = 0; j < 8; ++j) {
            const int i = i0 + j * 64 + lane, m = i / K, k = i - m * K;
            v[j] = (i < 32 * MB * K && m < M) ? a[(size_t)m * sm + (size_t)k * sk] : 0.f;
        }
#pragma unroll
        for (int j = 0; j < 8; ++j) {
            const int i = i0 + j * 64 + lane, m = i / K, k = i - m * K;
            if (i < 32 * MB * K) al[m * ld + k] = v[j];
        }
    }
    __syncthreads();
    for (int blk = blockIdx.x; blk < nblocks; blk += gridDim.x) {
        const int b = blk / blocks_per_img, p0 = (blk - b * blocks_per_img) * 64;
        const float* xb = x + (size_t)b * K * P;
        const int pa = min(p0 + li, P - 1), pb = min(p0 + 32 + li, P - 1);
        f32x16 acc[MB][2];
#pragma unroll
        for (int i = 0; i < MB; ++i)
#pragma unroll
            for (int j = 0; j < 2; ++j)
#pragma unroll
                for (int r = 0; r < 16; ++r) acc[i][j][r] = 0.f;
        for (int k0 = 0; k0 < K; k0 += 8) {
            float b0[4], b1[4];
#pragma unroll
            for (int s = 0; s < 4; ++s) {
                const float* row = xb + (size_t)(k0 + 2 * s + h) * P;
                b0[s] = row[pa];
                b1[s] = row[pb];
            }
#pragma unroll
            for (int s = 0; s < 4; ++s) {
#pragma unroll
                for (int i = 0; i < MB; ++i) {
                    const float av = al[(32 * i + li) * ld + k0 + 2 * s + h];
                    acc[i][0] = mfma32(av, b0[s], acc[i][0]);
                    acc[i][1] = mfma32(av, b1[s], acc[i][1]);
                }
            }
        }
        float* yb = y + (size_t)b * M * P;
#pragma unroll
        for (int i = 0; i < MB; ++i)
#pragma unroll
            for (int r = 0; r < 16; ++r) {
                const int m = 32 * i + acc_row(r) + 4 * h;
                if (m < M) {
                    if (p0 + li < P) yb[(size_t)m * P + p0 + li] = acc[i][0][r];
                    if (p0 + 32 + li < P) yb[(size_t)m * P + p0 + 32 + li] = acc[i][1][r];
                }
            }
    }
}

template <int COB, int CIB>
__global__ __launch_bounds__(64) void pw_wgrad_kernel(const float* __restrict__ dy, const float* __restrict__ x, int Co,
                                                       int Ci, int P, int nchunks, int chunks_per_img,
                                                       float* __restrict__ slabs) {
    extern __shared__ __attribute__((aligned(16))) float tl[];
    float* ty = tl;
    float* tx = tl + 32 * COB * 65;
    const int lane = threadIdx.x, li = lane & 31, h = lane >> 5;
    for (int i = lane; i < (32 * COB + 32 * CIB) * 65; i += 64) tl[i] = 0.f;
    f32x16 acc[COB][CIB];
#pragma unroll
    for (int i = 0; i < COB; ++i)
#pragma unroll
        for (int j = 0; j < CIB; ++j)
#pragma unroll
            for (int r = 0; r < 16; ++r) acc[i][j][r] = 0.f;
    for (int ch = blockIdx.x; ch < nchunks; ch += gridDim.x) {
        const int b = ch / chunks_per_img, p0 = (ch - b * chunks_per_img) * 64;
        const bool live = p0 + lane < P;
        const float* dyb = dy + (size_t)b * Co * P + p0 + lane;
        const float* xb = x + (size_t)b * Ci * P + p0 + lane;
        __syncthreads();
        auto stage = [&](const float* src, float* dst, int rows) {
            for (int r0 = 0; r0 < rows; r0 += 16) {
                float v[16];
#pragma unroll
                for (int j = 0; j < 16; ++j) v[j] = (live && r0 + j < rows) ? src[(size_t)(r0 + j) * P] : 0.f;
#pragma unroll
                for (int j = 0; j < 16; ++j)
                    if (r0 + j < rows) dst[(r0 + j) * 65 + lane] = v[j];
            }
        };
        stage(dyb, ty, Co);
        stage(xb, tx, Ci);
        __syncthreads();
#pragma unroll 4
        for (int s = 0; s < 32; ++s) {
            float av[COB], bv[CIB];
#pragma unroll
            for (int i = 0; i < COB; ++i) av[i] = ty[(32 * i + li) * 65 + 2 * s + h];
#pragma unroll
            for (int j = 0; j < CIB; ++j) bv[j] = tx[(32 * j + li) * 65 + 2 * s + h];
#pragma unroll
            for (int i = 0; i < COB; ++i)
#pragma unroll
                for (int j = 0; j < CIB; ++j) acc[i][j] = mfma32(av[i], bv[j], acc[i][j]);
        }
    }
    float* slab = slabs + (size_t)blockIdx.x * Co * Ci;
#pragma unroll
    for (int i = 0; i < COB; ++i)
#pragma unroll
        for (int j = 0; j < CIB; ++j)
#pragma unroll
            for (int r = 0; r < 16; ++r) {
                const int co = 32 * i + acc_row(r) + 4 * h, ci = 32 * j + li;
                if (co < Co && ci < Ci) slab[(size_t)co * Ci + ci] = acc[i][j][r];
            }
}

__global__ __launch_bounds__(256) void pw_slab_sum_kernel(const float* __restrict__ slabs, int nslab, int count,
                                                           float* __restrict__ dw) {
    const int i = blockIdx.x * 4 + (threadIdx.x >> 6), lane = threadIdx.x & 63;
    if (i >= count) return;
    float s0 = 0.f, s1 = 0.f;
    int k = lane;
    for (; k + 64 < nslab; k += 128) {
        s0 += slabs[(size_t)k * count + i];
        s1 += slabs[(size_t)(k + 64) * count + i];
    }
    if (k < nslab) s0 += slabs[(size_t)k * count + i];
    const float t = wave_sum(s0 + s1);
    if (lane == 0) dw[i] = t;
}

static int blocks_of(int n) { return ceil_div(n, 32); }
constexpr int PW_GRID = 256 * 8;

bool pwconv_supported(int Ci, int Co, int P) {
    (void)P;
    return Ci % 8 == 0 && Co % 8 == 0 && Ci <= 32 * PW_MAXB && Co <= 32 * PW_MAXB &&
           blocks_of(Ci) * blocks_of(Co) <= 8 && 32 * PW_MAXB * (Ci > Co ? Ci + 1 : Co + 1) * 4 <= 64 * 1024;
}

static int wgrad_slabs(int B, int P) {
    const int nchunks = B * ceil_div(P, 64);
    return nchunks < PW_GRID ? nchunks : PW_GRID;
}
size_t pwconv_bwd_workspace(int B, int Ci, int Co, int P) {
    return align_up((size_t)wgrad_slabs(B, P) * Co * Ci * sizeof(float), 256);
}

static hipError_t stream_launch(const float* a, int sm, int sk, int M, int K, const float* x, int B, int P, float* y,
                                hipStream_t stream) {
    const int bpi = ceil_div(P, 64), nblocks = B * bpi, grid = nblocks < PW_GRID ? nblocks : PW_GRID;
    const int mb = blocks_of(M);
    const size_t lds = (size_t)32 * mb * (K + 1) * sizeof(float);
#define PW_STREAM(MBV)                                                                                               \
    hipLaunchKernelGGL(pw_stream_kernel<MBV>, dim3(grid), dim3(64), lds, stream, a, sm, sk, M, K, x, P, nblocks, bpi, y)
    if (mb == 1) PW_STREAM(1);
    else if (mb == 2) PW_STREAM(2);
    else if (mb == 3) PW_STREAM(3);
    else PW_STREAM(4);
#undef PW_STREAM
    return hipGetLastError();
}

hipError_t pwconv_fwd_run(const float* x, const float* w, int B, int Ci, int Co, int P, float* y, hipStream_t stream) {
    return stream_launch(w, Ci, 1, Co, Ci, x, B, P, y, stream);
}

template <int COB>
static void wgrad_launch_ci(int cib, int grid, size_t lds, hipStream_t stream, const float* dy, const float* x, int Co,
                            int Ci, int P, int nchunks, int cpi, float* slabs) {
#define PW_WG(CIBV)                                                                                                    \
    hipLaunchKernelGGL((pw_wgrad_kernel<COB, CIBV>), dim3(grid), dim3(64), lds, stream, dy, x, Co, Ci, P, nchunks, cpi, \
                       slabs)
    if (cib == 1) PW_WG(1);
    else if (cib == 2) PW_WG(2);
    else if (cib == 3) { if constexpr (COB <= 2) PW_WG(3); }
    else { if constexpr (COB <= 2) PW_WG(4); }
#undef PW_WG
}

hipError_t pwconv_bwd_run(const float* dy, const float* x, const float* w, int B, int Ci, int Co, int P, float* dx,
                          float* dw, void* ws, hipStream_t stream) {
    if (dx) {
        hipError_t e = stream_launch(w, 1, Ci, Ci, Co, dy, B, P, dx, stream);
        if (e != hipSuccess) return e;
    }
    if (dw) {
        const int cpi = ceil_div(P, 64), nchunks = B * cpi, grid = wgrad_slabs(B, P);
        const int cob = blocks_of(Co), cib = blocks_of(Ci);
        const size_t lds = (size_t)(32 * cob + 32 * cib) * 65 * sizeof(float);
        float* slabs = static_cast<float*>(ws);
        if (cob == 1) wgrad_launch_ci<1>(cib, grid, lds, stream, dy, x, Co, Ci, P, nchunks, cpi, slabs);
        else if (cob == 2) wgrad_launch_ci<2>(cib, grid, lds, stream, dy, x, Co, Ci, P, nchunks, cpi, slabs);
        else if (cob == 3) wgrad_launch_ci<3>(cib, grid, lds, stream, dy, x, Co, Ci, P, nchunks, cpi, slabs);
        else wgrad_launch_ci<4>(cib, grid, lds, stream, dy, x, Co, Ci, P, nchunks, cpi, slabs);
        hipLaunchKernelGGL(pw_slab_sum_kernel, dim3(ceil_div(Co * Ci, 4)), dim3(256), 0, stream, slabs, grid, Co * Ci, dw);
    }
    return hipGetLastError();
}

}
```

cabinet_amd/functional.py:

```python

from __future__ import annotations

import ctypes as _ct

import torch
import torch.nn.functional as F

from . import _lib


def _ptr(t):
    return t.data_ptr() if t is not None else None


def _stream_handle(device):
    return torch.cuda.current_stream(device).cuda_stream


def _workspace(nbytes, device):
    if nbytes == 0:
        return None, 0
    ws = torch.empty(nbytes, dtype=torch.uint8, device=device)
    return ws, nbytes

# ... 1274 lines not shown

class _BnActDwConv(torch.autograd.Function):
    @staticmethod
    @torch.amp.custom_fwd(device_type="cuda", cast_inputs=torch.float32)
    def forward(fn_ctx, z, bn_w, bn_b, run_mean, run_var, conv_w, act, stride, training, momentum, eps):
        lib = _lib.load()
        z, bn_w, bn_b, cw = _f32c(z), _f32c(bn_w), _f32c(bn_b), _f32c(conv_w)
        B, C, H, W = z.shape
        K = cw.shape[-1]
        Ho, Wo = (H + 2 * (K // 2) - K) // stride + 1, (W + 2 * (K // 2) - K) // stride + 1
        y = torch.empty((B, C, Ho, Wo), dtype=torch.float32, device=z.device)
        mean = torch.empty(C, dtype=torch.float32, device=z.device)
        invstd = torch.empty(C, dtype=torch.float32, device=z.device)
        ws, nbytes = _workspace(lib.cabinet_bn_dwconv_fwd_workspace_bytes(B, C, H, W), z.device)
        with torch.cuda.device(z.device):
            rc = lib.cabinet_bn_dwconv_fwd(_ptr(z), _ptr(bn_w), _ptr(bn_b), _ptr(run_mean), _ptr(run_var), _ptr(cw), B, C,
                                           H, W, K, stride, act, int(training), float(momentum), float(eps), _ptr(y),
                                           _ptr(mean), _ptr(invstd), _ptr(ws), nbytes, _stream_handle(z.device))
        _lib.check(rc, "cabinet_bn_dwconv_fwd")
        fn_ctx.save_for_backward(z, bn_w, bn_b, cw, mean, invstd)
        fn_ctx.meta = (act, stride, bool(training))
        return y

    @staticmethod
    @torch.amp.custom_bwd(device_type="cuda")
    def backward(fn_ctx, g):
        lib = _lib.load()
        z, bn_w, bn_b, cw, mean, invstd = fn_ctx.saved_tensors
        act, stride, training = fn_ctx.meta
        g = _f32c(g)
        B, C, H, W = z.shape
        K = cw.shape[-1]
        dz, dbw, dbb, dcw = torch.empty_like(z), torch.empty_like(bn_w), torch.empty_like(bn_b), torch.empty_like(cw)
        ws, nbytes = _workspace(lib.cabinet_bn_dwconv_bwd_workspace_bytes(B, C, H, W, K, stride), z.device)
        with torch.cuda.device(z.device):
            rc = lib.cabinet_bn_dwconv_bwd(_ptr(g), _ptr(z), _ptr(bn_w), _ptr(bn_b), _ptr(mean), _ptr(invstd), _ptr(cw), B,
                                           C, H, W, K, stride, act, int(training), _ptr(dz), _ptr(dbw), _ptr(dbb),
                                           _ptr(dcw), _ptr(ws), nbytes, _stream_handle(z.device))
        _lib.check(rc, "cabinet_bn_dwconv_bwd")
        return dz, dbw, dbb, None, None, dcw, None, None, None, None, None


def bn_act_dwconv(z, bn, act, conv):
    if not z.is_cuda:
        raise RuntimeError("bn_act_dwconv: device tensors only")
    if act not in _ACT_CODES:
        raise RuntimeError(f"bn_act_dwconv: unknown activation {act!r}")
    training, momentum = _bn_step(bn)
    return _BnActDwConv.apply(z, bn.weight, bn.bias, bn.running_mean, bn.running_var, conv.weight, _ACT_CODES[act],
                              conv.stride[0], training, momentum, bn.eps)




def stem_conv_supported(conv):
    return (conv.in_channels == 3 and conv.out_channels == 64 and conv.kernel_size == (7, 7) and conv.stride == (2, 2)
            and conv.padding == (3, 3) and conv.dilation == (1, 1) and conv.groups == 1 and conv.bias is None
            and conv.padding_mode == "zeros")


class _StemConv(torch.autograd.Function):
    @staticmethod
    @torch.amp.custom_fwd(device_type="cuda", cast_inputs=torch.float32)
    def forward(fn_ctx, x, weight):
        lib = _lib.load()
        x, w = _f32c(x), _f32c(weight)
        B, _, H, W = x.shape
        y = torch.empty((B, 64, (H - 1) // 2 + 1, (W - 1) // 2 + 1), dtype=torch.float32, device=x.device)
        with torch.cuda.device(x.device):
            rc = lib.cabinet_stem_conv_fwd(_ptr(x), _ptr(w), B, H, W, _ptr(y), _stream_handle(x.device))
        _lib.check(rc, "cabinet_stem_conv_fwd")
        fn_ctx.save_for_backward(x, w)
        return y

    @staticmethod
    @torch.amp.custom_bwd(device_type="cuda")
    def backward(fn_ctx, g):
        lib = _lib.load()
        x, w = fn_ctx.saved_tensors
        g = _f32c(g)
        B, _, H, W = x.shape
        dx = None
        if fn_ctx.needs_input_grad[0]:
            dx = torch.ops.aten.convolution_backward(g, x, w, None, [2, 2], [3, 3], [1, 1], False, [0, 0], 1,
                                                     [True, False, False])[0]
        dw = torch.empty_like(w)
        ws, nbytes = _workspace(lib.cabinet_stem_conv_wrw_workspace_bytes(B, H, W), x.device)
        with torch.cuda.device(x.device):
            rc = lib.cabinet_stem_conv_wrw(_ptr(g), _ptr(x), B, H, W, _ptr(dw), _ptr(ws), nbytes,
                                           _stream_handle(x.device))
        _lib.check(rc, "cabinet_stem_conv_wrw")
        return dx, dw


def stem_conv(x, conv):
    if not x.is_cuda:
        raise RuntimeError("stem_conv: device tensors only")
    return _StemConv.apply(x, conv.weight)




def pwconv_supported(conv, x):
    if not (conv.kernel_size == (1, 1) and conv.stride == (1, 1) and conv.padding == (0, 0) and conv.groups == 1
            and conv.bias is None and conv.dilation == (1, 1)):
        return False
    P = x.shape[2] * x.shape[3]
    return (P >= 65536 and conv.in_channels <= 96 and conv.out_channels <= 96
            and bool(_lib.load().cabinet_pwconv_supported(conv.in_channels, conv.out_channels, P)))


class _PwConv(torch.autograd.Function):
    @staticmethod
    @torch.amp.custom_fwd(device_type="cuda", cast_inputs=torch.float32)
    def forward(fn_ctx, x, weight):
        lib = _lib.load()
        x = _f32c(x)
        Co, Ci = weight.shape[0], weight.shape[1]
        w2 = _f32c(weight).view(Co, Ci)
        B, P = x.shape[0], x.shape[2] * x.shape[3]
        y = torch.empty((B, Co) + tuple(x.shape[2:]), dtype=torch.float32, device=x.device)
        with torch.cuda.device(x.device):
            rc = lib.cabinet_pwconv_fwd(_ptr(x), _ptr(w2), B, Ci, Co, P, _ptr(y), _stream_handle(x.device))
        _lib.check(rc, "cabinet_pwconv_fwd")
        fn_ctx.save_for_backward(x, w2)
        fn_ctx.w_shape = weight.shape
        return y

    @staticmethod
    @torch.amp.custom_bwd(device_type="cuda")
    def backward(fn_ctx, g):
        lib = _lib.load()
        x, w2 = fn_ctx.saved_tensors
        g = _f32c(g)
        Co, Ci = w2.shape
        B, P = x.shape[0], x.shape[2] * x.shape[3]
        dx = torch.empty_like(x) if fn_ctx.needs_input_grad[0] else None
        dw = torch.empty_like(w2) if fn_ctx.needs_input_grad[1] else None
        ws, nbytes = _workspace(lib.cabinet_pwconv_bwd_workspace_bytes(B, Ci, Co, P), x.device)
        with torch.cuda.device(x.device):
            rc = lib.cabinet_pwconv_bwd(_ptr(g), _ptr(x), _ptr(w2), B, Ci, Co, P, _ptr(dx), _ptr(dw), _ptr(ws), nbytes,
                                        _stream_handle(x.device))
        _lib.check(rc, "cabinet_pwconv_bwd")
        return dx, (dw.view(fn_ctx.w_shape) if dw is not None else None)


def pwconv(x, conv):
    if not x.is_cuda:
        raise RuntimeError("pwconv: device tensors only")
    return _PwConv.apply(x, conv.weight)




PWCONV_WIDE_ENABLED = _os.environ.get("CABINET_PWCONV_WIDE", "1") != "0"


def pwconv_wide_supported(conv, x):
    if not (PWCONV_WIDE_ENABLED and isinstance(conv, torch.nn.Conv2d) and x.is_cuda and x.dim() == 4):
        return False
    if not (conv.kernel_size == (1, 1) and conv.stride == (1, 1) and conv.padding == (0, 0) and conv.groups == 1
            and conv.bias is None and conv.dilation == (1, 1)):
        return False
    if not (torch.is_grad_enabled() and conv.weight.requires_grad) or torch.is_autocast_enabled():
        return False
    if x.dtype != torch.float32 or conv.weight.dtype != torch.float32 or x.shape[0] < 1 or x.shape[2] * x.shape[3] < 1:
        return False
    return bool(_lib.load().cabinet_pwconv_wide_supported(conv.in_channels, conv.out_channels, x.shape[2] * x.shape[3]))


class _PwConvWide(torch.autograd.Function):

    @staticmethod
    def forward(fn_ctx, x, weight):
        x = x.contiguous()
        y = F.conv2d(x, weight)
        fn_ctx.save_for_backward(x, weight)
        return y

    @staticmethod
    def backward(fn_ctx, g):
        x, w = fn_ctx.saved_tensors
        g = g.contiguous()
        dx = None
        if fn_ctx.needs_input_grad[0]:
            dx = torch.ops.aten.convolution_backward(g, x, w, None, [1, 1], [0, 0], [1, 1], False, [0, 0], 1,
                                                     [True, False, False])[0]
        dw = None
        if fn_ctx.needs_input_grad[1]:
            lib = _lib.load()
            xc, gc = _f32c(x), _f32c(g)
            Co, Ci = w.shape[0], w.shape[1]
            B, P = xc.shape[0], xc.shape[2] * xc.shape[3]
            dw = torch.empty((Co, Ci, 1, 1), dtype=torch.float32, device=x.device)
            ws, nbytes = _workspace(lib.cabinet_pwconv_wide_wgrad_workspace_bytes(B, Ci, Co, P), x.device)
            with torch.cuda.device(x.device):
                rc = lib.cabinet_pwconv_wide_wgrad(_ptr(gc), _ptr(xc), B, Ci, Co, P, _ptr(dw), _ptr(ws), nbytes,
                                                   _stream_handle(x.device))
            _lib.check(rc, "cabinet_pwconv_wide_wgrad")
        return dx, dw


def pwconv_wide(x, conv):
    if not x.is_cuda:
        raise RuntimeError("pwconv_wide: device tensors only")
    return _PwConvWide.apply(x, conv.weight)




CONV3X3S2_ENABLED = _os.environ.get("CABINET_CONV3X3S2", "1") != "0"


def conv3x3s2_supported(conv, x):
    if not (CONV3X3S2_ENABLED and isinstance(conv, torch.nn.Conv2d) and x.is_cuda and x.dim() == 4):
        return False
    if not (conv.kernel_size == (3, 3) and conv.stride == (2, 2) and conv.padding == (1, 1) and conv.groups == 1
            and conv.bias is None and conv.dilation == (1, 1) and conv.padding_mode == "zeros"):
        return False
    if not (torch.is_grad_enabled() and conv.weight.requires_grad) or torch.is_autocast_enabled():
        return False
    if x.dtype != torch.float32 or conv.weight.dtype != torch.float32 or x.shape[0] < 1 or x.shape[2] * x.shape[3] < 1:
        return False
    return x.shape[1] == conv.in_channels and bool(_lib.load().cabinet_conv3x3s2_supported(conv.in_channels, conv.out_channels))


def _conv3x3s2_native_wgrad(Ci, B, H):
    return Ci == 3 and B * (((H - 1) // 2 + 1 + 3) // 4) >= 1024


class _Conv3x3S2(torch.autograd.Function):

    @staticmethod
    def forward(fn_ctx, x, weight):
        x = x.contiguous()
        y = F.conv2d(x, weight, None, 2, 1)
        fn_ctx.save_for_backward(x, weight)
        return y

    @staticmethod
    def backward(fn_ctx, g):
        x, w = fn_ctx.saved_tensors
        g = g.contiguous()
        lib = _lib.load()
        xc, gc = _f32c(x), _f32c(g)
        Co, Ci = w.shape[0], w.shape[1]
        B, H, W = xc.shape[0], xc.shape[2], xc.shape[3]
        cb = torch.ops.aten.convolution_backward
        dx = None
        if fn_ctx.needs_input_grad[0] and Ci == 64:
            dx = torch.empty_like(xc)
            with torch.cuda.device(x.device):
                rc = lib.cabinet_conv3x3s2_dgrad(_ptr(gc), _ptr(_f32c(w)), B, Ci, Co, H, W, _ptr(dx), _stream_handle(x.device))
            _lib.check(rc, "cabinet_conv3x3s2_dgrad")
        elif fn_ctx.needs_input_grad[0]:
            dx = cb(g, x, w, None, [2, 2], [1, 1], [1, 1], False, [0, 0], 1, [True, False, False])[0]
        dw = None
        if fn_ctx.needs_input_grad[1] and _conv3x3s2_native_wgrad(Ci, B, H):
            dw = torch.empty((Co, Ci, 3, 3), dtype=torch.float32, device=x.device)
            ws, nbytes = _workspace(lib.cabinet_conv3x3s2_wgrad_workspace_bytes(B, Ci, Co, H, W), x.device)
            with torch.cuda.device(x.device):
                rc = lib.cabinet_conv3x3s2_wgrad(_ptr(gc), _ptr(xc), B, Ci, Co, H, W, _ptr(dw), _ptr(ws), nbytes,
                                                 _stream_handle(x.device))
            _lib.check(rc, "cabinet_conv3x3s2_wgrad")
        elif fn_ctx.needs_input_grad[1]:
            dw = cb(g, x, w, None, [2, 2], [1, 1], [1, 1], False, [0, 0], 1, [False, True, False])[1]
        return dx, dw


class Conv2dS2(torch.nn.Conv2d):

    def _conv_forward(self, input, weight, bias):
        if bias is None and conv3x3s2_supported(self, input):
            return _Conv3x3S2.apply(input, weight)
        return super()._conv_forward(input, weight, bias)




def eval_chip_accum_supported(logits, chip_size, flip=False):
    if not (logits.is_cuda and logits.dim() == 4 and _lib.available()):
        return False
    _, C, hl, wl = logits.shape
    return bool(_lib.load().cabinet_eval_chip_accum_supported(C, hl, wl, int(chip_size[0]), int(chip_size[1]), int(bool(flip))))


def eval_chip_accum(dst, logits, logits_flipped, chip_size, origin, rcp_y=None, rcp_x=None):
    lib = _lib.load()
    if not (dst.is_cuda and dst.dtype == torch.float32 and dst.is_contiguous()):
        raise RuntimeError("eval_chip_accum: dst must be a dense fp32 device tensor")
    a = _f32c(logits)
    b = _f32c(logits_flipped) if logits_flipped is not None else None
    if b is not None and b.shape != a.shape:
        raise RuntimeError("eval_chip_accum: the flipped chip's logits must have the shape of the chip's")
    N, C, hl, wl = a.shape
    if dst.shape[:2] != (N, C):
        raise RuntimeError(f"eval_chip_accum: dst {tuple(dst.shape)} does not match logits {tuple(a.shape)}")
    FH, FW = dst.shape[2:]
    ry = _f32c(rcp_y) if rcp_y is not None else None
    rx = _f32c(rcp_x) if rcp_x is not None else None
    if (ry is not None and ry.numel() != FH) or (rx is not None and rx.numel() != FW):
        raise RuntimeError("eval_chip_accum: rcp_y / rcp_x must have one entry per row / column of dst")
    dev = dst.device
    with torch.cuda.device(dev):
        rc = lib.cabinet_eval_chip_accum(_ptr(a), _ptr(b), N, C, hl, wl, int(chip_size[0]), int(chip_size[1]), _ptr(dst), FH, FW,
                                         int(origin[0]), int(origin[1]), _ptr(ry), _ptr(rx), _stream_handle(dev))
# ... 49 lines not shown
```

cabinet_amd/models/mobilenetv3.py:

```python

from __future__ import annotations

import math
from pathlib import Path

import torch
import torch.nn as nn

__all__ = ["MobileNetV3", "InvertedResidual", "SELayer", "HardSwish", "HardSigmoid",
           "mobilenetv3_large", "mobilenetv3_small"]


def _make_divisible(v, divisor, min_value=None):
    floor = divisor if min_value is None else min_value
    rounded = max(floor, int(v + divisor / 2) // divisor * divisor)
    return rounded + divisor if rounded < 0.9 * v else rounded


class HardSigmoid(nn.Module):

    def __init__(self, inplace: bool = True) -> None:
        super().__init__()
        self.relu = nn.ReLU6(inplace=inplace)

    def forward(self, x):
        return self.relu(x + 3) / 6


class HardSwish(nn.Module):

    def __init__(self, inplace: bool = True) -> None:
        super().__init__()
        self.sigmoid = HardSigmoid(inplace=inplace)

    def forward(self, x):
        return x * self.sigmoid(x)


class SELayer(nn.Module):

    def __init__(self, channel, reduction=4):
        super().__init__()
        squeezed = _make_divisible(channel // reduction, 8)
        self.avg_pool = nn.AdaptiveAvgPool2d(1)
        self.fc = nn.Sequential(nn.Linear(channel, squeezed), nn.ReLU(inplace=True),
                                nn.Linear(squeezed, channel), HardSigmoid())

    def gate(self, x):
        n, c = x.shape[:2]
        return self.fc(self.avg_pool(x).view(n, c))

    def forward(self, x):
        n, c = x.shape[:2]
        return x * self.gate(x).view(n, c, 1, 1)


def _act(use_hs):
    return HardSwish() if use_hs else nn.ReLU(inplace=True)


class _FusedSequential(nn.Sequential):

    def forward(self, x, residual=None):
        if not x.is_cuda:
            y = super().forward(x)
            return y if residual is None else residual + y
        from ..functional import (bn_act, bn_act_dwconv, dwconv, dwconv_supported, gate_act, pwconv,
                                  pwconv_supported, pwconv_wide, pwconv_wide_supported, se_tail)

        layers = [m for m in self if not isinstance(m, nn.Identity)]

        def act_of(m):
            return "relu" if isinstance(m, nn.ReLU) else "hardswish" if isinstance(m, HardSwish) else None

        i = 0
        while i < len(layers):
            m = layers[i]
            nxt = layers[i + 1] if i + 1 < len(layers) else None
            if isinstance(m, nn.BatchNorm2d) and isinstance(nxt, SELayer):
                act = act_of(layers[i + 2]) if i + 2 < len(layers) else None
                x, i = se_tail(x, m, nxt, act), i + (3 if act else 2)
            elif isinstance(m, nn.BatchNorm2d):
                act = act_of(nxt)
                nxt2 = layers[i + 2] if act and i + 2 < len(layers) else None
                if isinstance(nxt2, nn.Conv2d) and nxt2.groups > 1 and dwconv_supported(nxt2):
                    x, i = bn_act_dwconv(x, m, act, nxt2), i + 3
                else:
                    last = i + (2 if act else 1) >= len(layers)
                    x, i = bn_act(x, m, act, residual if last else None), i + (2 if act else 1)
                    if last:
                        residual = None
            elif isinstance(m, SELayer):
                act = act_of(nxt)
                x, i = gate_act(x, m.gate(x), act), i + (2 if act else 1)
            elif isinstance(m, nn.Conv2d) and m.groups == 1 and pwconv_supported(m, x):
                x, i = pwconv(x, m), i + 1
            elif isinstance(m, nn.Conv2d) and m.groups > 1 and dwconv_supported(m):
                x, i = dwconv(x, m), i + 1
            elif pwconv_wide_supported(m, x):
                x, i = pwconv_wide(x, m), i + 1
            else:
                x, i = m(x), i + 1
        return x if residual is None else residual + x


def conv_3x3_bn(inp, oup, stride):
    from ..functional import Conv2dS2

    return _FusedSequential(Conv2dS2(inp, oup, 3, stride, 1, bias=False), nn.BatchNorm2d(oup), HardSwish())


def conv_1x1_bn(inp, oup):
    return _FusedSequential(nn.Conv2d(inp, oup, 1, 1, 0, bias=False), nn.BatchNorm2d(oup), HardSwish())


class InvertedResidual(nn.Module):

    def __init__(self, inp, hidden_dim, oup, kernel_size, stride, use_se, use_hs):
        super().__init__()
        if stride not in (1, 2):
            raise ValueError(f"stride must be 1 or 2, got {stride}")
        self.identity = stride == 1 and inp == oup
        pad = (kernel_size - 1) // 2

        def depthwise():
            return nn.Conv2d(hidden_dim, hidden_dim, kernel_size, stride, pad, groups=hidden_dim, bias=False)

        layers = []
        if inp == hidden_dim:
            layers += [depthwise(), nn.BatchNorm2d(hidden_dim), _act(use_hs)]
            layers += [SELayer(hidden_dim) if use_se else nn.Identity()]
        else:
            layers += [nn.Conv2d(inp, hidden_dim, 1, 1, 0, bias=False), nn.BatchNorm2d(hidden_dim), _act(use_hs)]
            layers += [depthwise(), nn.BatchNorm2d(hidden_dim)]
            layers += [SELayer(hidden_dim) if use_se else nn.Identity(), _act(use_hs)]
        layers += [nn.Conv2d(hidden_dim, oup, 1, 1, 0, bias=False), nn.BatchNorm2d(oup)]
        self.conv = _FusedSequential(*layers)

    def forward(self, x):
        if self.identity:
            return self.conv(x, residual=x)
        return self.conv(x)


class MobileNetV3(nn.Module):

    def __init__(self, cfgs, mode, num_classes=1000, width_mult=1.0, weights=None):
        super().__init__()
        self.cfgs = cfgs
        self.weights = weights
        if mode not in ("large", "small"):
            raise ValueError(f"mode must be 'large' or 'small', got '{mode}'")
        cin = _make_divisible(16 * width_mult, 8)
        stages = [conv_3x3_bn(3, cin, 2)]
        exp = cin
        for k, t, c, use_se, use_hs, s in self.cfgs:
            cout = _make_divisible(c * width_mult, 8)
            exp = _make_divisible(cin * t, 8)
            stages.append(InvertedResidual(cin, exp, cout, k, s, use_se, use_hs))
            cin = cout
        self.features = nn.Sequential(*stages)
        self.conv = conv_1x1_bn(cin, exp)
        self.avgpool = nn.AdaptiveAvgPool2d((1, 1))
        head = {"large": 1280, "small": 1024}[mode]
        if width_mult > 1.0:
            head = _make_divisible(head * width_mult, 8)
        self.classifier = nn.Sequential(nn.Linear(exp, head), HardSwish(), nn.Dropout(0.2),
                                        nn.Linear(head, num_classes))
        self._initialize_weights()

    def forward(self, x):
        return self.conv(self.features(x))

    def _initialize_weights(self):
        if self.weights is not None and Path(self.weights).is_file():
            try:
                loaded = torch.load(self.weights, map_location="cpu", weights_only=True)
                merged = self.state_dict()
                merged.update({k: v for k, v in loaded.items() if "classifier" not in k})
                self.load_state_dict(merged)
                print(f"Loaded pretrained weights from {self.weights}")
                return
            except Exception as e:
                print(f"Failed to load backbone weights from {self.weights}: {e}")
                print("Proceeding with random weight initialization.")
        for m in self.modules():
            if isinstance(m, nn.Conv2d):
                fan = m.kernel_size[0] * m.kernel_size[1] * m.out_channels
                m.weight.data.normal_(0, math.sqrt(2.0 / fan))
                if m.bias is not None:
                    m.bias.data.zero_()
            elif isinstance(m, nn.BatchNorm2d):
                m.weight.data.fill_(1)
                m.bias.data.zero_()
            elif isinstance(m, nn.Linear):
                m.weight.data.normal_(0, 0.01)
                m.bias.data.zero_()


def mobilenetv3_large(**kwargs):
    from .constants import MOBILENETV3_CFGS

    return MobileNetV3(MOBILENETV3_CFGS["large"], mode="large", **kwargs)


def mobilenetv3_small(**kwargs):
    from .constants import MOBILENETV3_CFGS

    return MobileNetV3(MOBILENETV3_CFGS["small"], mode="small", **kwargs)
```

include/cabinet_hip.h:

```cpp
#ifndef CABINET_HIP_H_
#define CABINET_HIP_H_

#include <stddef.h>

#ifdef __cplusplus
extern "C" {
#endif

#define CABINET_ABI_VERSION 8

#define CABINET_OK 0
#define CABINET_ERR_INVALID_ARG (-1)
#define CABINET_ERR_UNSUPPORTED (-2)
#define CABINET_ERR_WORKSPACE (-3)
#define CABINET_ERR_HIP (-4)

typedef void* cabinet_stream_t;

int cabinet_abi_version(void);
const char* cabinet_last_error(void);

#define CABINET_PREC_FP32 0
#define CABINET_PREC_BF16X3 1
#define CABINET_PREC_BF16X6 2
// ... 89 lines not shown
                               int B, int C, int Hl, int Wl, int H, int W, float thresh, int ignore_lb,
                               float* loss_px, float* blk_sum, int* blk_cnt,
                               const float* class_weight_a, const float* class_weight_b, cabinet_stream_t stream);
int cabinet_ohem_up_pair_w_bwd(const float* logits_low_a, const float* logits_low_b, const long long* labels,
                               const float* loss_px, int B, int C, int Hl, int Wl, int H, int W, float thresh, int ignore_lb,
                               float coef, float* dlogits_low, void* workspace, size_t workspace_bytes,
                               const float* class_weight_a, const float* class_weight_b, cabinet_stream_t stream);
size_t cabinet_ohem_select_workspace_bytes(int nheads, int B, int H, int W);
int cabinet_ohem_select(const float* loss_px, const long long* labels, const double* stats, int nheads,
                        int B, int C, int H, int W, float thresh, int n_min_a, int n_min_b, int ignore_lb,
                        const float* class_weight_a, const float* class_weight_b, double* sel,
                        void* workspace, size_t workspace_bytes, cabinet_stream_t stream);
int cabinet_ohem_up_w_bwd_sel(const float* logits_low, const long long* labels, const float* loss_px,
                              int B, int C, int Hl, int Wl, int H, int W, const double* sel, int ignore_lb, float coef,
                              float* dlogits_low, void* workspace, size_t workspace_bytes, const float* class_weight,
                              cabinet_stream_t stream);
int cabinet_ohem_up_pair_w_bwd_sel(const float* logits_low_a, const float* logits_low_b, const long long* labels,
                                   const float* loss_px, int B, int C, int Hl, int Wl, int H, int W, const double* sel,
                                   int ignore_lb, float coef, float* dlogits_low, void* workspace, size_t workspace_bytes,
                                   const float* class_weight_a, const float* class_weight_b, cabinet_stream_t stream);

int cabinet_cab_local_supported(int B, int C, int H, int W);
size_t cabinet_cab_local_fwd_workspace_bytes(int B, int C, int H, int W);
size_t cabinet_cab_local_bwd_workspace_bytes(int B, int C, int H, int W);
int cabinet_cab_local_fwd(const float* x, const float* glob, const float* gamma,
                          const float* const* dw_w, const float* const* bn_weight, const float* const* bn_bias,
                          float* const* running_mean, float* const* running_var,
                          int B, int C, int H, int W, int training, float momentum, float eps,
                          float* out, float* save_mean, float* save_invstd,
                          void* workspace, size_t workspace_bytes, cabinet_stream_t stream);
int cabinet_cab_local_bwd(const float* dout, const float* x, const float* glob, const float* gamma,
                          const float* const* dw_w, const float* const* bn_weight, const float* const* bn_bias,
                          const float* save_mean, const float* save_invstd,
                          int B, int C, int H, int W, int training,
                          float* dx, float* dglob, float* dgamma_part,
                          float* const* ddw_w, float* const* dbn_weight, float* const* dbn_bias,
                          void* workspace, size_t workspace_bytes, cabinet_stream_t stream);

int cabinet_cab_qkv_supported(int B, int C, int Kc, int Vc, int H, int W, int n_sizes, const int* sizes);
int cabinet_cab_qkv_padded_bins(int n_sizes, const int* sizes);
size_t cabinet_cab_qkv_fwd_workspace_bytes(int B, int C, int Kc, int Vc, int H, int W, int n_sizes, const int* sizes);
int cabinet_cab_qkv_fwd(const float* x, const float* wq, const float* wk, const float* wv,
                        const float* bnq_weight, const float* bnq_bias, float* bnq_running_mean, float* bnq_running_var,
                        const float* bnk_weight, const float* bnk_bias, float* bnk_running_mean, float* bnk_running_var,
                        const float* wpk, const float* wpv,
                        int B, int C, int Kc, int Vc, int H, int W, int n_sizes, const int* sizes,
                        int training, float momentum, float eps,
                        float* q, float* k, float* v,
                        float* zqk, float* vv, float* kk, float* pooled_k, float* pooled_v,
                        float* save_mean, float* save_invstd,
                        void* workspace, size_t workspace_bytes, cabinet_stream_t stream);
size_t cabinet_cab_qkv_bwd_workspace_bytes(int B, int C, int Kc, int Vc, int H, int W, int n_sizes, const int* sizes);
int cabinet_cab_qkv_bwd(const float* dq, const float* dk, const float* dv, const float* x,
                        const float* wq, const float* wk, const float* wv,
                        const float* bnq_weight, const float* bnq_bias, const float* bnk_weight, const float* bnk_bias,
                        const float* wpk, const float* wpv,
                        const float* zqk, const float* vv, const float* kk, const float* pooled_k,
                        const float* pooled_v, const float* save_mean, const float* save_invstd,
                        int B, int C, int Kc, int Vc, int H, int W, int n_sizes, const int* sizes, int training,
                        float* dx, float* dwqk, float* dwv,
                        float* dbnq_weight, float* dbnq_bias, float* dbnk_weight, float* dbnk_bias,
                        float* dwpk, float* dwpv,
                        void* workspace, size_t workspace_bytes, cabinet_stream_t stream);

size_t cabinet_conv1x1_fwd_workspace_bytes(int Ci, int Co);
int cabinet_conv1x1_fwd(const float* x, const float* w, int B, int Ci, int Co, int P, float* y,
                        void* workspace, size_t workspace_bytes, cabinet_stream_t stream);
int cabinet_conv1x1_bias_supported(int B, int Ci, int Co, int P);
int cabinet_conv1x1_bias_fwd(const float* x, const float* w, const float* bias , int B, int Ci, int Co, int P, float* y,
                             void* workspace, size_t workspace_bytes, cabinet_stream_t stream);
int cabinet_channel_sum(const float* d , int B, int C, int P, float* out , cabinet_stream_t stream);
size_t cabinet_conv1x1_bwd_workspace_bytes(int B, int Ci, int Co, int P);
int cabinet_conv1x1_bwd(const float* dy, const float* x, const float* w, int B, int Ci, int Co, int P,
                        float* dx, float* dw, void* workspace, size_t workspace_bytes, cabinet_stream_t stream);

size_t cabinet_bn_act_workspace_bytes(int B, int C, int P);
int cabinet_bn_act_fwd(const float* x, const float* weight, const float* bias,
                       float* running_mean, float* running_var, const float* residual ,
                       int B, int C, int P, int act, int training, float momentum, float eps,
                       float* y, float* save_mean, float* save_invstd,
                       void* workspace, size_t workspace_bytes, cabinet_stream_t stream);
int cabinet_bn_act_fwd_part(const float* x, const float* conv_part, const float* weight, const float* bias,
                            float* running_mean, float* running_var, const float* residual ,
                            int B, int C, int H, int W, int act, int training, float momentum, float eps,
                            float* y, float* save_mean, float* save_invstd, cabinet_stream_t stream);
int cabinet_bn_act_bwd(const float* dy, const float* x, const float* weight, const float* bias,
                       const float* save_mean, const float* save_invstd,
                       int B, int C, int P, int act, int training,
                       float* dx, float* dweight, float* dbias,
                       void* workspace, size_t workspace_bytes, cabinet_stream_t stream);

int cabinet_bn_cls_supported(int C, int K, int P);
int cabinet_bn_cls_table_floats(int C, int K);
size_t cabinet_bn_cls_fwd_workspace_bytes(int B, int C, int P);
int cabinet_bn_cls_fwd(const float* z, const float* conv_part , const float* bn_weight, const float* bn_bias,
                       float* running_mean, float* running_var, const float* w_cls , const float* bias ,
                       int B, int C, int K, int H, int W, int training, float momentum, float eps,
                       float* y , float* table,
                       void* workspace, size_t workspace_bytes, cabinet_stream_t stream);
size_t cabinet_bn_cls_bwd_workspace_bytes(int B, int C, int K, int P);
int cabinet_bn_cls_bwd(const float* dy , const float* z, const float* table,
                       int B, int C, int K, int H, int W, int training,
                       float* dz, float* dbn_weight, float* dbn_bias, float* dw_cls, float* dbias ,
                       void* workspace, size_t workspace_bytes, cabinet_stream_t stream);

int cabinet_dwconv_supported(int K, int stride);
int cabinet_dwconv_fwd(const float* x, const float* weight, int B, int C, int H, int W, int K, int stride,
                       float* y, cabinet_stream_t stream);
size_t cabinet_dwconv_bwd_workspace_bytes(int B, int C, int H, int W, int K, int stride);
int cabinet_dwconv_bwd(const float* dy, const float* x, const float* weight, int B, int C, int H, int W, int K,
                       int stride, float* dx, float* dw, void* workspace, size_t workspace_bytes,
                       cabinet_stream_t stream);

int cabinet_gate_act_fwd(const float* x, const float* gate, int B, int C, int P, int act, float* y,
                         cabinet_stream_t stream);
size_t cabinet_gate_act_bwd_workspace_bytes(int B, int C, int P);
int cabinet_gate_act_bwd(const float* dy, const float* x, const float* gate, int B, int C, int P, int act,
                         float* dx, float* dgate, void* workspace, size_t workspace_bytes, cabinet_stream_t stream);

size_t cabinet_se_act_bwd_workspace_bytes(int B, int C, int P);
int cabinet_se_act_bwd_reduce(const float* dy, const float* z, const float* mean, const float* invstd, const float* bn_weight,
                              const float* bn_bias, const float* gate, const float* a2, int B, int C, int P, int act,
                              float* sums, float* da2, void* workspace, size_t workspace_bytes, cabinet_stream_t stream);
int cabinet_se_act_bwd_coef(const float* sums, const float* gate, const float* ds, int B, int C, int P, int training,
                            float* dbn_weight, float* dbn_bias, float* coef, float* ds_over_p, cabinet_stream_t stream);
int cabinet_se_act_bwd_dx(const float* dy, const float* z, const float* mean, const float* invstd, const float* bn_weight,
                          const float* bn_bias, const float* gate, const float* ds_over_p, const float* coef,
                          int B, int C, int P, int act, float* dz, cabinet_stream_t stream);

size_t cabinet_bn_dwconv_fwd_workspace_bytes(int B, int C, int H, int W);
int cabinet_bn_dwconv_fwd(const float* z, const float* bn_weight, const float* bn_bias,
                          float* running_mean, float* running_var, const float* conv_weight,
                          int B, int C, int H, int W, int K, int stride, int act, int training,
                          float momentum, float eps, float* y, float* save_mean, float* save_invstd,
                          void* workspace, size_t workspace_bytes, cabinet_stream_t stream);
size_t cabinet_bn_dwconv_bwd_workspace_bytes(int B, int C, int H, int W, int K, int stride);
int cabinet_bn_dwconv_bwd(const float* dy, const float* z, const float* bn_weight, const float* bn_bias,
                          const float* save_mean, const float* save_invstd, const float* conv_weight,
                          int B, int C, int H, int W, int K, int stride, int act, int training,
                          float* dz, float* dbn_weight, float* dbn_bias, float* dconv_weight,
                          void* workspace, size_t workspace_bytes, cabinet_stream_t stream);

int cabinet_stem_conv_fwd(const float* x, const float* weight, int B, int H, int W, float* y, cabinet_stream_t stream);
size_t cabinet_stem_conv_wrw_workspace_bytes(int B, int H, int W);
int cabinet_stem_conv_wrw(const float* dy, const float* x, int B, int H, int W, float* dw,
                          void* workspace, size_t workspace_bytes, cabinet_stream_t stream);

int cabinet_pwconv_supported(int Ci, int Co, int P);
int cabinet_pwconv_fwd(const float* x, const float* w, int B, int Ci, int Co, int P, float* y, cabinet_stream_t stream);
size_t cabinet_pwconv_bwd_workspace_bytes(int B, int Ci, int Co, int P);
int cabinet_pwconv_bwd(const float* dy, const float* x, const float* w, int B, int Ci, int Co, int P,
                       float* dx, float* dw, void* workspace, size_t workspace_bytes, cabinet_stream_t stream);

int cabinet_pwconv_wide_supported(int Ci, int Co, int P);
size_t cabinet_pwconv_wide_wgrad_workspace_bytes(int B, int Ci, int Co, int P);
int cabinet_pwconv_wide_wgrad(const float* dy, const float* x, int B, int Ci, int Co, int P, float* dw,
                              void* workspace, size_t workspace_bytes, cabinet_stream_t stream);

int cabinet_conv3x3_supported(int C0, int C1, int Co);
int cabinet_conv3x3_tile_blocks(int B, int H, int W);
size_t cabinet_conv3x3_fwd_workspace_bytes(int B, int C0, int C1, int Co, int H, int W);
int cabinet_conv3x3_fwd(const float* x0, const float* x1, const float* w, int B, int C0, int C1, int Co, int H, int W,
                        float* y, float* bn_part, void* workspace, size_t workspace_bytes, cabinet_stream_t stream);
size_t cabinet_conv3x3_bwd_workspace_bytes(int B, int C0, int C1, int Co, int H, int W);
int cabinet_conv3x3_bwd(const float* dy, const float* x0, const float* x1, const float* w, int B, int C0, int C1, int Co,
                        int H, int W, float* dx0, float* dx1, float* dw,
                        void* workspace, size_t workspace_bytes, cabinet_stream_t stream);

int cabinet_eval_chip_accum_supported(int C, int hl, int wl, int ch, int cw, int flip);
int cabinet_eval_chip_accum(const float* a, const float* b, int N, int C, int hl, int wl, int ch, int cw, float* dst, int FH, int FW,
                            int y0, int x0, const float* rcp_y, const float* rcp_x, cabinet_stream_t stream);
int cabinet_eval_scale_merge(const float* prob, int N, int C, int FH, int FW, int hst, int hed, int wst, int wed, float* total, int H,
                             int W, cabinet_stream_t stream);
int cabinet_eval_argmax_hist(const float* total, const long long* labels, int N, int C, int H, int W, int ignore_lb, long long* hist,
                             unsigned char* pred, cabinet_stream_t stream);

int cabinet_conv3x3s2_supported(int Ci, int Co);
size_t cabinet_conv3x3s2_wgrad_workspace_bytes(int B, int Ci, int Co, int H, int W);
int cabinet_conv3x3s2_wgrad(const float* dy, const float* x, int B, int Ci, int Co, int H, int W, float* dw,
                            void* workspace, size_t workspace_bytes, cabinet_stream_t stream);
int cabinet_conv3x3s2_dgrad(const float* dy, const float* w, int B, int Ci, int Co, int H, int W, float* dx,
                            cabinet_stream_t stream);

#ifdef __cplusplus
}
#endif
#endif
```

Before: 356.6 images/s.

## Fuse pointwise-conv backward with BN/activation (and depthwise) backward

Adds a new pw_bn_bwd kernel path that fuses the 1x1 convolution backward with the BatchNorm+activation backward. It also adds a variant that folds in the following depthwise conv backward. The BN backward helper is split into sums, finalize and dx stages so the BN coefficient application can be merged into the pwconv dgrad/wgrad instead of writing and rereading an intermediate dz tensor. The MobileNetV3 block dispatcher routes conv→BN→act(→dwconv) sequences to these fused autograd functions when shapes are supported. This adds kernel complexity and more routing conditions.

```diff
diff --git a/cabinet_amd/_lib.py b/cabinet_amd/_lib.py
--- a/cabinet_amd/_lib.py
+++ b/cabinet_amd/_lib.py
@@ -84,6 +84,12 @@
     "cabinet_pwconv_fwd": (_INT, [_PTR] * 2 + [_INT] * 4 + [_PTR] + [_PTR]),
     "cabinet_pwconv_bwd_workspace_bytes": (_SZ, [_INT] * 4),
     "cabinet_pwconv_bwd": (_INT, [_PTR] * 3 + [_INT] * 4 + [_PTR] * 2 + [_PTR, _SZ, _PTR]),
+    "cabinet_pw_bn_bwd_supported": (_INT, [_INT] * 4),
+    "cabinet_pw_bn_bwd_workspace_bytes": (_SZ, [_INT] * 4),
+    "cabinet_pw_bn_bwd": (_INT, [_PTR] * 8 + [_INT] * 6 + [_PTR] * 4 + [_PTR, _SZ, _PTR]),
+    "cabinet_pw_bn_dwconv_bwd_supported": (_INT, [_INT] * 7),
+    "cabinet_pw_bn_dwconv_bwd_workspace_bytes": (_SZ, [_INT] * 7),
+    "cabinet_pw_bn_dwconv_bwd": (_INT, [_PTR] * 9 + [_INT] * 9 + [_PTR] * 5 + [_PTR, _SZ, _PTR]),
     "cabinet_pwconv_wide_supported": (_INT, [_INT] * 3),
     "cabinet_pwconv_wide_wgrad_workspace_bytes": (_SZ, [_INT] * 4),
     "cabinet_pwconv_wide_wgrad": (_INT, [_PTR] * 2 + [_INT] * 4 + [_PTR] + [_PTR, _SZ, _PTR]),
diff --git a/cabinet_amd/build.py b/cabinet_amd/build.py
--- a/cabinet_amd/build.py
+++ b/cabinet_amd/build.py
@@ -15,7 +15,7 @@
 LIB_PATH = os.path.join(PKG_DIR, "libcabinet_hip.so")
 ARCH = "gfx950"
 
-SOURCES = ["capi.hip", "cab_attn_fwd.hip", "cab_attn_bf16.hip", "cab_attn_bwd.hip", "ffm.hip", "ffm_bwd_fused.hip", "ffm_bwd_adj.hip", "ffm_fwd_fused.hip", "gemm_bf16.hip", "ohem.hip", "cab_local.hip", "cab_local_tiled.hip", "cab_qkv.hip", "cab_qkv_fused.hip", "bn_act.hip", "dwconv.hip", "stem_conv.hip", "pwconv.hip", "pwconv_wide.hip", "conv3x3_s2.hip", "small_gemm.hip", "conv3x3_wino.hip", "bn_cls.hip", "eval_tail.hip"]
+SOURCES = ["capi.hip", "cab_attn_fwd.hip", "cab_attn_bf16.hip", "cab_attn_bwd.hip", "ffm.hip", "ffm_bwd_fused.hip", "ffm_bwd_adj.hip", "ffm_fwd_fused.hip", "gemm_bf16.hip", "ohem.hip", "cab_local.hip", "cab_local_tiled.hip", "cab_qkv.hip", "cab_qkv_fused.hip", "bn_act.hip", "dwconv.hip", "stem_conv.hip", "pwconv.hip", "pw_bn_bwd.hip", "pwconv_wide.hip", "conv3x3_s2.hip", "small_gemm.hip", "conv3x3_wino.hip", "bn_cls.hip", "eval_tail.hip"]
 HEADERS = ["common.hpp", "cab_local.hpp", "cab_qkv.hpp", "blocks.hpp", "act.hpp", "bn_finalize.hpp", "slab_sum.hpp", os.path.join("..", "..", "include", "cabinet_hip.h")]
 
 
diff --git a/cabinet_amd/csrc/act.hpp b/cabinet_amd/csrc/act.hpp
--- a/cabinet_amd/csrc/act.hpp
+++ b/cabinet_amd/csrc/act.hpp
@@ -34,9 +34,13 @@
 size_t bn_act_workspace(int B, int C, int P);
 hipError_t bn_stats_run(const float* x, float* running_mean, float* running_var, int B, int C, int P, int training,
                         float momentum, float eps, float* save_mean, float* save_invstd, void* ws, hipStream_t stream);
-hipError_t bn_bwd_tail_run(const float* part, int nt, const float* dy, const float* x, const float* weight,
-                           const float* bias, const float* save_mean, const float* save_invstd, int B, int C, int P,
-                           int act, int training, float* dx, float* dweight, float* dbias, float* coef,
-                           hipStream_t stream);
+hipError_t bn_bwd_finalize_run(const float* part, int nt, int B, int C, int P, int training, float* dweight, float* dbias,
+                               float* coef, hipStream_t stream);
+hipError_t bn_bwd_sums_run(const float* dy, const float* x, const float* weight, const float* bias, const float* save_mean,
+                           const float* save_invstd, int B, int C, int P, int act, int training, float* dweight,
+                           float* dbias, void* ws, const float** coef_out, hipStream_t stream);
+hipError_t bn_bwd_dx_run(const float* dy, const float* x, const float* weight, const float* bias, const float* save_mean,
+                         const float* save_invstd, const float* coef, int B, int C, int P, int act, float* dx,
+                         hipStream_t stream);
 
 }
diff --git a/cabinet_amd/csrc/bn_act.hip b/cabinet_amd/csrc/bn_act.hip
--- a/cabinet_amd/csrc/bn_act.hip
+++ b/cabinet_amd/csrc/bn_act.hip
@@ -391,28 +391,42 @@
     return hipGetLastError();
 }
 
-hipError_t bn_bwd_tail_run(const float* part, int nt, const float* dy, const float* x, const float* weight,
-                           const float* bias, const float* save_mean, const float* save_invstd, int B, int C, int P,
-                           int act, int training, float* dx, float* dweight, float* dbias, float* coef,
-                           hipStream_t stream) {
-    const int chunks = ba_chunks(P), grid = B * C * chunks;
+hipError_t bn_bwd_finalize_run(const float* part, int nt, int B, int C, int P, int training, float* dweight, float* dbias,
+                               float* coef, hipStream_t stream) {
     hipLaunchKernelGGL(bn_act_bwd_finalize_kernel, dim3(C), dim3(BA_T), 0, stream, part, nt, C, (double)B * (double)P,
                        training, dweight, dbias, coef);
-    hipLaunchKernelGGL(bn_act_bwd_dx_kernel, dim3(grid), dim3(BA_T), 0, stream, dy, x, save_mean, save_invstd, weight,
-                       bias, coef, C, P, chunks, act, dx);
-    return hipGetLastError();
-}
-
-hipError_t bn_act_bwd_run(const float* dy, const float* x, const float* weight, const float* bias,
-                          const float* save_mean, const float* save_invstd, int B, int C, int P, int act, int training,
-                          float* dx, float* dweight, float* dbias, void* ws, hipStream_t stream) {
+    return hipGetLastError();
+}
+
+hipError_t bn_bwd_sums_run(const float* dy, const float* x, const float* weight, const float* bias, const float* save_mean,
+                           const float* save_invstd, int B, int C, int P, int act, int training, float* dweight,
+                           float* dbias, void* ws, const float** coef_out, hipStream_t stream) {
     const int chunks = ba_chunks(P), grid = B * C * chunks, nt = B * chunks;
     float* part = static_cast<float*>(ws);
     float* coef = reinterpret_cast<float*>(static_cast<char*>(ws) + align_up((size_t)2 * C * nt * sizeof(float), 256));
     hipLaunchKernelGGL(bn_act_bwd_reduce_kernel, dim3(grid), dim3(BA_T), 0, stream, dy, x, save_mean, save_invstd, weight,
                        bias, B, C, P, chunks, act, part);
-    return bn_bwd_tail_run(part, nt, dy, x, weight, bias, save_mean, save_invstd, B, C, P, act, training, dx, dweight,
-                           dbias, coef, stream);
+    *coef_out = coef;
+    return bn_bwd_finalize_run(part, nt, B, C, P, training, dweight, dbias, coef, stream);
+}
+
+hipError_t bn_bwd_dx_run(const float* dy, const float* x, const float* weight, const float* bias, const float* save_mean,
+                         const float* save_invstd, const float* coef, int B, int C, int P, int act, float* dx,
+                         hipStream_t stream) {
+    const int chunks = ba_chunks(P), grid = B * C * chunks;
+    hipLaunchKernelGGL(bn_act_bwd_dx_kernel, dim3(grid), dim3(BA_T), 0, stream, dy, x, save_mean, save_invstd, weight,
+                       bias, coef, C, P, chunks, act, dx);
+    return hipGetLastError();
+}
+
+hipError_t bn_act_bwd_run(const float* dy, const float* x, const float* weight, const float* bias,
+                          const float* save_mean, const float* save_invstd, int B, int C, int P, int act, int training,
+                          float* dx, float* dweight, float* dbias, void* ws, hipStream_t stream) {
+    const float* coef = nullptr;
+    hipError_t e = bn_bwd_sums_run(dy, x, weight, bias, save_mean, save_invstd, B, C, P, act, training, dweight, dbias, ws, &coef,
+                                   stream);
+    if (e != hipSuccess) return e;
+    return bn_bwd_dx_run(dy, x, weight, bias, save_mean, save_invstd, coef, B, C, P, act, dx, stream);
 }
 
 size_t gate_act_workspace(int rows, int P) { return align_up((size_t)rows * ba_chunks(P) * sizeof(float), 256); }
diff --git a/cabinet_amd/csrc/capi.hip b/cabinet_amd/csrc/capi.hip
--- a/cabinet_amd/csrc/capi.hip
+++ b/cabinet_amd/csrc/capi.hip
@@ -109,6 +109,15 @@
 hipError_t stem_conv_fwd_run(const float* x, const float* w, int B, int H, int W, float* y, hipStream_t stream);
 hipError_t stem_conv_wrw_run(const float* dy, const float* x, int B, int H, int W, float* dw, void* ws,
                              hipStream_t stream);
+size_t pw_bn_bwd_workspace(int B, int Ci, int Co, int P);
+size_t pw_bn_dwconv_bwd_workspace(int B, int Ci, int C, int H, int W, int K);
+hipError_t pw_bn_bwd_run(const float* g, const float* z, const float* x, const float* w, const float* bn_w, const float* bn_b,
+                         const float* save_mean, const float* save_invstd, int B, int Ci, int Co, int P, int act, int training,
+                         float* dx, float* dw, float* dbn_w, float* dbn_b, void* ws, hipStream_t stream);
+hipError_t pw_bn_dwconv_bwd_run(const float* dy, const float* z, const float* x, const float* w, const float* bn_w,
+                                const float* bn_b, const float* save_mean, const float* save_invstd, const float* dw_w, int B,
+                                int Ci, int C, int H, int W, int K, int S, int act, int training, float* dx, float* dw,
+                                float* dbn_w, float* dbn_b, float* ddw_w, void* ws, hipStream_t stream);
 bool pwconv_wide_supported(int Ci, int Co, int P);
 size_t pwconv_wide_wgrad_workspace(int B, int Ci, int Co, int P);
 hipError_t pwconv_wide_wgrad_run(const float* dy, const float* x, int B, int Ci, int Co, int P, float* dw, void* ws,
@@ -1118,7 +1127,7 @@
 static int check_pwconv(int B, int Ci, int Co, int P, const char* who) {
     if (B <= 0 || Ci <= 0 || Co <= 0 || P <= 0) return fail(CABINET_ERR_INVALID_ARG, "%s: non-positive dimension", who);
     if (!cabinet::pwconv_supported(Ci, Co, P))
-        return fail(CABINET_ERR_UNSUPPORTED, "%s: Ci=%d, Co=%d (multiples of 8, <= 120, block product <= 8)", who, Ci, Co);
+        return fail(CABINET_ERR_UNSUPPORTED, "%s: Ci=%d, Co=%d (multiples of 8, <= 128, block product <= 8)", who, Ci, Co);
     return CABINET_OK;
 }
 
@@ -1147,6 +1156,77 @@
         return fail(CABINET_ERR_WORKSPACE, "pwconv_bwd: workspace %zu < %zu bytes", workspace_bytes, need);
     return hip_status(cabinet::pwconv_bwd_run(dy, x, w, B, Ci, Co, P, dx, dw, workspace, static_cast<hipStream_t>(stream)),
                       "pwconv_bwd launch");
+}
+
+static bool pw_bn_shape_ok(int B, int Ci, int Co, int P) {
+    return B > 0 && Ci > 0 && Co > 0 && P > 0 && cabinet::pwconv_supported(Ci, Co, P) && P <= (1 << 27) &&
+           (long long)B * ((P + 63) / 64) <= (1LL << 30);
+}
+static int check_pw_bn(int B, int Ci, int Co, int P, int act, const char* who) {
+    if (int rc = check_bn_act(B, Co, P, act, who)) return rc;
+    if (Ci <= 0) return fail(CABINET_ERR_INVALID_ARG, "%s: non-positive dimension", who);
+    if (!pw_bn_shape_ok(B, Ci, Co, P))
+        return fail(CABINET_ERR_UNSUPPORTED, "%s: Ci=%d, Co=%d, B=%d, P=%d (channels: multiples of 8, <= 128, block product <= 8; P <= 2^27)",
+                    who, Ci, Co, B, P);
+    return CABINET_OK;
+}
+
+int cabinet_pw_bn_bwd_supported(int B, int Ci, int Co, int P) { return pw_bn_shape_ok(B, Ci, Co, P) ? 1 : 0; }
+
+size_t cabinet_pw_bn_bwd_workspace_bytes(int B, int Ci, int Co, int P) {
+    return pw_bn_shape_ok(B, Ci, Co, P) ? cabinet::pw_bn_bwd_workspace(B, Ci, Co, P) : 0;
+}
+
+int cabinet_pw_bn_bwd(const float* dy, const float* z, const float* x, const float* conv_weight, const float* bn_weight,
+                      const float* bn_bias, const float* save_mean, const float* save_invstd, int B, int Ci, int Co, int P,
+                      int act, int training, float* dx, float* dconv_weight, float* dbn_weight, float* dbn_bias,
+                      void* workspace, size_t workspace_bytes, cabinet_stream_t stream) {
+    if (int rc = check_pw_bn(B, Ci, Co, P, act, "pw_bn_bwd")) return rc;
+    if (!dy || !z || !x || !conv_weight || !bn_weight || !bn_bias || !save_mean || !save_invstd || !dconv_weight ||
+        !dbn_weight || !dbn_bias)
+        return fail(CABINET_ERR_INVALID_ARG, "pw_bn_bwd: null tensor pointer");
+    CABINET_REQUIRE_ALIGNED("pw_bn_bwd", dy, z, x, dx);
+    const size_t need = cabinet::pw_bn_bwd_workspace(B, Ci, Co, P);
+    if (!workspace || workspace_bytes < need)
+        return fail(CABINET_ERR_WORKSPACE, "pw_bn_bwd: workspace %zu < %zu bytes", workspace_bytes, need);
+    return hip_status(cabinet::pw_bn_bwd_run(dy, z, x, conv_weight, bn_weight, bn_bias, save_mean, save_invstd, B, Ci, Co, P,
+                                             act, training, dx, dconv_weight, dbn_weight, dbn_bias, workspace,
+                                             static_cast<hipStream_t>(stream)),
+                      "pw_bn_bwd launch");
+}
+
+int cabinet_pw_bn_dwconv_bwd_supported(int B, int Ci, int C, int H, int W, int K, int stride) {
+    return H > 0 && W > 0 && (long long)H * W <= (1 << 27) && cabinet::dwconv_supported(K, stride) &&
+                   pw_bn_shape_ok(B, Ci, C, H * W)
+               ? 1
+               : 0;
+}
+
+size_t cabinet_pw_bn_dwconv_bwd_workspace_bytes(int B, int Ci, int C, int H, int W, int K, int stride) {
+    return cabinet_pw_bn_dwconv_bwd_supported(B, Ci, C, H, W, K, stride) ? cabinet::pw_bn_dwconv_bwd_workspace(B, Ci, C, H, W, K)
+                                                                         : 0;
+}
+
+int cabinet_pw_bn_dwconv_bwd(const float* dy, const float* z, const float* x, const float* conv_weight,
+                             const float* bn_weight, const float* bn_bias, const float* save_mean, const float* save_invstd,
+                             const float* dw_weight, int B, int Ci, int C, int H, int W, int K, int stride, int act,
+                             int training, float* dx, float* dconv_weight, float* dbn_weight, float* dbn_bias,
+                             float* ddw_weight, void* workspace, size_t workspace_bytes, cabinet_stream_t stream) {
+    if (int rc = check_dwconv(B, C, H, W, K, stride, "pw_bn_dwconv_bwd")) return rc;
+    if (int rc = check_pw_bn(B, Ci, C, H * W, act, "pw_bn_dwconv_bwd")) return rc;
+    if (!dy || !z || !x || !conv_weight || !bn_weight || !bn_bias || !save_mean || !save_invstd || !dw_weight ||
+        !dconv_weight || !dbn_weight || !dbn_bias || !ddw_weight)
+        return fail(CABINET_ERR_INVALID_ARG, "pw_bn_dwconv_bwd: null tensor pointer");
+    CABINET_REQUIRE_ALIGNED("pw_bn_dwconv_bwd", z, x, dx);
+    const size_t need = cabinet::pw_bn_dwconv_bwd_workspace(B, Ci, C, H, W, K);
+    if (!workspace || workspace_bytes < need || (reinterpret_cast<uintptr_t>(workspace) & 15))
+        return fail(CABINET_ERR_WORKSPACE, "pw_bn_dwconv_bwd: workspace %zu < %zu bytes, or not 16-byte aligned",
+                    workspace_bytes, need);
+    return hip_status(cabinet::pw_bn_dwconv_bwd_run(dy, z, x, conv_weight, bn_weight, bn_bias, save_mean, save_invstd,
+                                                    dw_weight, B, Ci, C, H, W, K, stride, act, training, dx, dconv_weight,
+                                                    dbn_weight, dbn_bias, ddw_weight, workspace,
+                                                    static_cast<hipStream_t>(stream)),
+                      "pw_bn_dwconv_bwd launch");
 }
 
 int cabinet_pwconv_wide_supported(int Ci, int Co, int P) {
diff --git a/cabinet_amd/csrc/dwconv.hip b/cabinet_amd/csrc/dwconv.hip
--- a/cabinet_amd/csrc/dwconv.hip
+++ b/cabinet_amd/csrc/dwconv.hip
@@ -401,10 +401,10 @@
     return fwd_dispatch(z, w, s, K, S, BnFold{save_mean, save_invstd, bn_w, bn_b, act}, y, stream);
 }
 
-hipError_t bn_dwconv_bwd_run(const float* dy, const float* z, const float* bn_w, const float* bn_b,
-                             const float* save_mean, const float* save_invstd, const float* w, int B, int C, int H,
-                             int W, int K, int S, int act, int training, float* dz, float* dbn_w, float* dbn_b,
-                             float* dw, void* ws, hipStream_t stream) {
+hipError_t bn_dwconv_bwd_sums_run(const float* dy, const float* z, const float* bn_w, const float* bn_b,
+                                  const float* save_mean, const float* save_invstd, const float* w, int B, int C, int H,
+                                  int W, int K, int S, int act, int training, float* dbn_w, float* dbn_b, float* dw,
+                                  void* ws, const float** da_out, const float** coef_out, hipStream_t stream) {
     const BnDwWs L = bn_dw_layout(B, C, H, W, K);
     char* base = static_cast<char*>(ws);
     auto at = [&](size_t o) { return reinterpret_cast<float*>(base + o); };
@@ -413,8 +413,20 @@
     hipError_t e = bwd_dispatch(dy, z, w, s, K, S, BnFold{save_mean, save_invstd, bn_w, bn_b, act}, at(L.da), dw,
                                 at(L.part), at(L.bnpart), stream);
     if (e != hipSuccess) return e;
-    return bn_bwd_tail_run(at(L.bnpart), B * bwd_tiles(H, W), at(L.da), z, bn_w, bn_b, save_mean, save_invstd, B, C,
-                           H * W, act, training, dz, dbn_w, dbn_b, at(L.coef), stream);
-}
-
-}
+    *da_out = at(L.da);
+    *coef_out = at(L.coef);
+    return bn_bwd_finalize_run(at(L.bnpart), B * bwd_tiles(H, W), B, C, H * W, training, dbn_w, dbn_b, at(L.coef), stream);
+}
+
+hipError_t bn_dwconv_bwd_run(const float* dy, const float* z, const float* bn_w, const float* bn_b,
+                             const float* save_mean, const float* save_invstd, const float* w, int B, int C, int H,
+                             int W, int K, int S, int act, int training, float* dz, float* dbn_w, float* dbn_b,
+                             float* dw, void* ws, hipStream_t stream) {
+    const float *da = nullptr, *coef = nullptr;
+    hipError_t e = bn_dwconv_bwd_sums_run(dy, z, bn_w, bn_b, save_mean, save_invstd, w, B, C, H, W, K, S, act, training, dbn_w,
+                                          dbn_b, dw, ws, &da, &coef, stream);
+    if (e != hipSuccess) return e;
+    return bn_bwd_dx_run(da, z, bn_w, bn_b, save_mean, save_invstd, coef, B, C, H * W, act, dz, stream);
+}
+
+}
diff --git a/cabinet_amd/csrc/pw_bn_bwd.hip b/cabinet_amd/csrc/pw_bn_bwd.hip
--- /dev/null
+++ b/cabinet_amd/csrc/pw_bn_bwd.hip
@@ -0,0 +1,281 @@
+#include <type_traits>
+
+#include "act.hpp"
+#include "common.hpp"
+
+namespace cabinet {
+
+constexpr int PBB_T = 256;
+constexpr int PBB_PX = 32;
+constexpr int PBB_LD = 33;
+constexpr int PBB_CHUNK = 64;
+constexpr int PBB_GRID = 512;
+
+__host__ __device__ constexpr int pbb_regs(int CO8, int CI8) {
+    const int cob = (CO8 + 3) / 4, cib = (CI8 + 3) / 4;
+    return 16 * cob * cib + 16 + 4 * (2 * CO8 + CI8) + 48;
+}
+
+template <bool VEC>
+__device__ __forceinline__ f32x4 pbb_load4(const float* __restrict__ rows, const int (&o)[4]) {
+    if (VEC) return *reinterpret_cast<const f32x4*>(rows + o[0]);
+    f32x4 v;
+#pragma unroll
+    for (int e = 0; e < 4; ++e) v[e] = rows[o[e]];
+    return v;
+}
+
+template <int CO8, int CI8, bool EXACT>
+__global__ __launch_bounds__(PBB_T, pbb_regs(CO8, CI8) > 240 ? 1 : 2) void pw_bn_bwd_kernel(
+    const float* __restrict__ g, const float* __restrict__ z, const float* __restrict__ x, const float* __restrict__ w,
+    const float* __restrict__ mean, const float* __restrict__ invstd, const float* __restrict__ gamma,
+    const float* __restrict__ beta, const float* __restrict__ coef, int Co, int Ci, int P, int nchunks, int cpi, int nslab,
+    int act, float* __restrict__ dx, float* __restrict__ slabs) {
+    constexpr int COB = (CO8 + 3) / 4, CIB = (CI8 + 3) / 4, COR = 8 * CO8, CIR = 8 * CI8, LDW = COR + 1;
+    constexpr bool PF = pbb_regs(CO8, CI8) <= 240;
+    extern __shared__ __attribute__((aligned(16))) float lds[];
+    float* chn = lds;
+    float* wl = lds + COR * 8;
+    float* tiles = wl + 32 * CIB * LDW;
+    const int wave = __builtin_amdgcn_readfirstlane(threadIdx.x >> 6), lane = threadIdx.x & 63, li = lane & 31, h = lane >> 5;
+    const int q4 = (lane & 7) * 4, rr = lane >> 3;
+    float* ty = tiles + wave * (COR + CIR) * PBB_LD;
+    float* tx = ty + COR * PBB_LD;
+    const int co8 = EXACT ? CO8 : Co >> 3, ci8 = EXACT ? CI8 : Ci >> 3;
+    const int soff = 4 * h * P + li;
+
+    for (int c = threadIdx.x; c < COR; c += PBB_T) {
+        const bool live = c < Co;
+        const float gam = live ? gamma[c] : 0.f, inv = live ? invstd[c] : 0.f;
+        chn[c * 8 + 0] = live ? mean[c] : 0.f;
+        chn[c * 8 + 1] = inv;
+        chn[c * 8 + 2] = gam;
+        chn[c * 8 + 3] = live ? beta[c] : 0.f;
+        chn[c * 8 + 4] = live ? coef[c] : 0.f;
+        chn[c * 8 + 5] = live ? coef[Co + c] : 0.f;
+        chn[c * 8 + 6] = gam * inv;
+        chn[c * 8 + 7] = 0.f;
+    }
+    if (dx)
+        for (int i = threadIdx.x; i < 32 * CIB * COR; i += PBB_T) {
+            const int ci = i / COR, co = i - ci * COR;
+            wl[ci * LDW + co] = (ci < Ci && co < Co) ? w[(size_t)co * Ci + ci] : 0.f;
+        }
+    if (!EXACT)
+        for (int i = lane; i < (COR + CIR) * PBB_LD; i += 64) ty[i] = 0.f;
+    __syncthreads();
+
+    f32x16 acc[COB][CIB];
+#pragma unroll
+    for (int i = 0; i < COB; ++i)
+#pragma unroll
+        for (int j = 0; j < CIB; ++j)
+#pragma unroll
+            for (int r = 0; r < 16; ++r) acc[i][j][r] = 0.f;
+
+    f32x4 pg[CO8], pz[CO8], px[CI8];
+    const int wid = blockIdx.x * 4 + wave;
+    auto chunk_of = [&](int u) { return wid < nslab ? wid + (u >> 1) * nslab : nchunks; };
+    auto issue = [&](int u, auto vec_tag) {
+        constexpr bool VEC = decltype(vec_tag)::value;
+        const int ch = chunk_of(u), b = ch / cpi, p0 = (ch - b * cpi) * PBB_CHUNK + (u & 1) * PBB_PX, p = p0 + q4;
+        int o[4];
+#pragma unroll
+        for (int e = 0; e < 4; ++e) o[e] = rr * P + (VEC ? min(p, P - 4) : min(p + e, P - 1)) - p0;
+        const float* gb = g + (size_t)b * Co * P + p0;
+        const float* zb = z + (size_t)b * Co * P + p0;
+        const float* xb = x + (size_t)b * Ci * P + p0;
+#pragma unroll
+        for (int j = 0; j < CO8; ++j)
+            if (j < co8) {
+                pg[j] = pbb_load4<VEC>(gb + (size_t)(8 * j) * P, o);
+                pz[j] = pbb_load4<VEC>(zb + (size_t)(8 * j) * P, o);
+            }
+#pragma unroll
+        for (int j = 0; j < CI8; ++j)
+            if (j < ci8) px[j] = pbb_load4<VEC>(xb + (size_t)(8 * j) * P, o);
+    };
+
+    auto run = [&](auto vec_tag) {
+    if (PF && chunk_of(0) < nchunks) issue(0, vec_tag);
+    for (int u = 0; chunk_of(u) < nchunks; ++u) {
+        const int ch = chunk_of(u), b = ch / cpi, p0 = (ch - b * cpi) * PBB_CHUNK + (u & 1) * PBB_PX;
+        if (!PF) issue(u, vec_tag);
+#pragma unroll
+        for (int j = 0; j < CO8; ++j)
+            if (j < co8) {
+                const f32x4 c0 = *reinterpret_cast<const f32x4*>(chn + (8 * j + rr) * 8);
+                const f32x4 c1 = *reinterpret_cast<const f32x4*>(chn + (8 * j + rr) * 8 + 4);
+                const float mu = c0[0], inv = c0[1], gam = c0[2], bet = c0[3], m1 = c1[0], m2 = c1[1], gi = c1[2];
+                float* dst = ty + (8 * j + rr) * PBB_LD + q4;
+#pragma unroll
+                for (int e = 0; e < 4; ++e) {
+                    const float xh = (pz[j][e] - mu) * inv;
+                    const float du = pg[j][e] * act_grad(fmaf(xh, gam, bet), act);
+                    dst[e] = gi * (du - m1 - xh * m2);
+                }
+            }
+#pragma unroll
+        for (int j = 0; j < CI8; ++j)
+            if (j < ci8) {
+                float* dst = tx + (8 * j + rr) * PBB_LD + q4;
+#pragma unroll
+                for (int e = 0; e < 4; ++e) dst[e] = p0 + q4 + e < P ? px[j][e] : 0.f;
+            }
+        if (PF && chunk_of(u + 1) < nchunks) issue(u + 1, vec_tag);
+        __builtin_amdgcn_fence(__ATOMIC_RELEASE, "wavefront");
+        __builtin_amdgcn_wave_barrier();
+        __builtin_amdgcn_fence(__ATOMIC_ACQUIRE, "wavefront");
+        if (dx) {
+            const int kmax = EXACT ? COR : Co;
+            float* dxb = dx + (size_t)b * Ci * P + p0;
+#pragma unroll
+            for (int i = 0; i < CIB; ++i) {
+                f32x16 ax;
+#pragma unroll
+                for (int r = 0; r < 16; ++r) ax[r] = 0.f;
+                const float* wr = wl + (32 * i + li) * LDW + h;
+                for (int k0 = 0; k0 < kmax; k0 += 2) ax = mfma32(wr[k0], ty[(k0 + h) * PBB_LD + li], ax);
+                if (p0 + li < P) {
+#pragma unroll
+                    for (int r = 0; r < 16; ++r) {
+                        const int ci = 32 * i + acc_row(r) + 4 * h;
+                        if (ci < Ci) (dxb + (size_t)(32 * i + acc_row(r)) * P)[soff] = ax[r];
+                    }
+                }
+            }
+        }
+        int ra[COB], rb[CIB];
+#pragma unroll
+        for (int i = 0; i < COB; ++i) ra[i] = min(32 * i + li, COR - 1) * PBB_LD + h;
+#pragma unroll
+        for (int j = 0; j < CIB; ++j) rb[j] = min(32 * j + li, CIR - 1) * PBB_LD + h;
+#pragma unroll 4
+        for (int s = 0; s < PBB_PX / 2; ++s) {
+            float av[COB], bv[CIB];
+#pragma unroll
+            for (int i = 0; i < COB; ++i) av[i] = ty[ra[i] + 2 * s];
+#pragma unroll
+            for (int j = 0; j < CIB; ++j) bv[j] = tx[rb[j] + 2 * s];
+#pragma unroll
+            for (int i = 0; i < COB; ++i)
+#pragma unroll
+                for (int j = 0; j < CIB; ++j) acc[i][j] = mfma32(av[i], bv[j], acc[i][j]);
+        }
+        __builtin_amdgcn_fence(__ATOMIC_RELEASE, "wavefront");
+        __builtin_amdgcn_wave_barrier();
+        __builtin_amdgcn_fence(__ATOMIC_ACQUIRE, "wavefront");
+    }
+
+    };
+    if ((P & 3) == 0) run(std::true_type{});
+    else run(std::false_type{});
+
+    if (wid < nslab) {
+        float* slab = slabs + (size_t)wid * Co * Ci;
+#pragma unroll
+        for (int i = 0; i < COB; ++i)
+#pragma unroll
+            for (int j = 0; j < CIB; ++j)
+#pragma unroll
+                for (int r = 0; r < 16; ++r) {
+                    const int co = 32 * i + acc_row(r) + 4 * h, ci = 32 * j + li;
+                    if (co < Co && ci < Ci) slab[(size_t)co * Ci + ci] = acc[i][j][r];
+                }
+    }
+}
+
+hipError_t pw_slab_sum_run(const float* slabs, int nslab, int count, float* dw, hipStream_t stream);
+
+static int pbb_slabs(int B, int P) {
+    const long long nchunks = (long long)B * ceil_div(P, PBB_CHUNK);
+    return nchunks < 4 * PBB_GRID ? (int)nchunks : 4 * PBB_GRID;
+}
+size_t pw_bn_bwd_slab_bytes(int B, int Ci, int Co, int P) {
+    return align_up((size_t)pbb_slabs(B, P) * Co * Ci * sizeof(float), 256);
+}
+
+template <int CO8, int CI8, bool EXACT>
+static hipError_t pbb_launch(const float* g, const float* z, const float* x, const float* w, const float* mean,
+                             const float* invstd, const float* gamma, const float* beta, const float* coef, int B, int Ci,
+                             int Co, int P, int act, float* dx, float* dw, float* slabs, hipStream_t stream) {
+    constexpr int CIB = (CI8 + 3) / 4, COR = 8 * CO8, CIR = 8 * CI8;
+    constexpr size_t lds = ((size_t)COR * 8 + (size_t)32 * CIB * (COR + 1) + (size_t)4 * (COR + CIR) * PBB_LD) * sizeof(float);
+    static_assert(lds <= 160 * 1024, "pw_bn_bwd: the tile does not fit the LDS");
+    static lds_attr_mask mask{0};
+    if (hipError_t e = ensure_dynamic_lds(reinterpret_cast<const void*>(pw_bn_bwd_kernel<CO8, CI8, EXACT>), lds, mask);
+        e != hipSuccess)
+        return e;
+    const int cpi = ceil_div(P, PBB_CHUNK), nchunks = B * cpi, nslab = pbb_slabs(B, P);
+    hipLaunchKernelGGL((pw_bn_bwd_kernel<CO8, CI8, EXACT>), dim3(ceil_div(nslab, 4)), dim3(PBB_T), lds, stream, g, z, x, w, mean,
+                       invstd, gamma, beta, coef, Co, Ci, P, nchunks, cpi, nslab, act, dx, slabs);
+    return pw_slab_sum_run(slabs, nslab, Co * Ci, dw, stream);
+}
+
+hipError_t pw_bn_bwd_fused_run(const float* g, const float* z, const float* x, const float* w, const float* mean,
+                               const float* invstd, const float* gamma, const float* beta, const float* coef, int B, int Ci,
+                               int Co, int P, int act, float* dx, float* dw, float* slabs, hipStream_t stream) {
+#define PBB_ARGS g, z, x, w, mean, invstd, gamma, beta, coef, B, Ci, Co, P, act, dx, dw, slabs, stream
+    if (Co == 16 && Ci == 16) return pbb_launch<2, 2, true>(PBB_ARGS);
+    if (Co == 64 && Ci == 16) return pbb_launch<8, 2, true>(PBB_ARGS);
+    if (Co == 24 && Ci == 64) return pbb_launch<3, 8, true>(PBB_ARGS);
+    if (Co == 72 && Ci == 24) return pbb_launch<9, 3, true>(PBB_ARGS);
+    if (Co == 24 && Ci == 72) return pbb_launch<3, 9, true>(PBB_ARGS);
+    const int cob = ceil_div(Co, 32), cib = ceil_div(Ci, 32);
+#define PBB_GEN(A, Bv) \
+    if (cob == A && cib == Bv) return pbb_launch<4 * A, 4 * Bv, false>(PBB_ARGS)
+    PBB_GEN(1, 1);
+    PBB_GEN(1, 2);
+    PBB_GEN(1, 3);
+    PBB_GEN(1, 4);
+    PBB_GEN(2, 1);
+    PBB_GEN(2, 2);
+    PBB_GEN(2, 3);
+    PBB_GEN(2, 4);
+    PBB_GEN(3, 1);
+    PBB_GEN(3, 2);
+    PBB_GEN(4, 1);
+    PBB_GEN(4, 2);
+#undef PBB_GEN
+#undef PBB_ARGS
+    return hipErrorInvalidValue;
+}
+
+size_t bn_dwconv_bwd_workspace(int B, int C, int H, int W, int K);
+hipError_t bn_dwconv_bwd_sums_run(const float* dy, const float* z, const float* bn_w, const float* bn_b,
+                                  const float* save_mean, const float* save_invstd, const float* w, int B, int C, int H,
+                                  int W, int K, int S, int act, int training, float* dbn_w, float* dbn_b, float* dw,
+                                  void* ws, const float** da_out, const float** coef_out, hipStream_t stream);
+
+size_t pw_bn_bwd_workspace(int B, int Ci, int Co, int P) {
+    return align_up(bn_act_workspace(B, Co, P), 256) + pw_bn_bwd_slab_bytes(B, Ci, Co, P);
+}
+size_t pw_bn_dwconv_bwd_workspace(int B, int Ci, int C, int H, int W, int K) {
+    return align_up(bn_dwconv_bwd_workspace(B, C, H, W, K), 256) + pw_bn_bwd_slab_bytes(B, Ci, C, H * W);
+}
+
+hipError_t pw_bn_bwd_run(const float* g, const float* z, const float* x, const float* w, const float* bn_w, const float* bn_b,
+                         const float* save_mean, const float* save_invstd, int B, int Ci, int Co, int P, int act, int training,
+                         float* dx, float* dw, float* dbn_w, float* dbn_b, void* ws, hipStream_t stream) {
+    const float* coef = nullptr;
+    hipError_t e = bn_bwd_sums_run(g, z, bn_w, bn_b, save_mean, save_invstd, B, Co, P, act, training, dbn_w, dbn_b, ws, &coef,
+                                   stream);
+    if (e != hipSuccess) return e;
+    float* slabs = reinterpret_cast<float*>(static_cast<char*>(ws) + align_up(bn_act_workspace(B, Co, P), 256));
+    return pw_bn_bwd_fused_run(g, z, x, w, save_mean, save_invstd, bn_w, bn_b, coef, B, Ci, Co, P, act, dx, dw, slabs, stream);
+}
+
+hipError_t pw_bn_dwconv_bwd_run(const float* dy, const float* z, const float* x, const float* w, const float* bn_w,
+                                const float* bn_b, const float* save_mean, const float* save_invstd, const float* dw_w, int B,
+                                int Ci, int C, int H, int W, int K, int S, int act, int training, float* dx, float* dw,
+                                float* dbn_w, float* dbn_b, float* ddw_w, void* ws, hipStream_t stream) {
+    const float *da = nullptr, *coef = nullptr;
+    hipError_t e = bn_dwconv_bwd_sums_run(dy, z, bn_w, bn_b, save_mean, save_invstd, dw_w, B, C, H, W, K, S, act, training,
+                                          dbn_w, dbn_b, ddw_w, ws, &da, &coef, stream);
+    if (e != hipSuccess) return e;
+    float* slabs = reinterpret_cast<float*>(static_cast<char*>(ws) + align_up(bn_dwconv_bwd_workspace(B, C, H, W, K), 256));
+    return pw_bn_bwd_fused_run(da, z, x, w, save_mean, save_invstd, bn_w, bn_b, coef, B, Ci, C, H * W, act, dx, dw, slabs,
+                               stream);
+}
+
+}
diff --git a/cabinet_amd/csrc/pwconv.hip b/cabinet_amd/csrc/pwconv.hip
--- a/cabinet_amd/csrc/pwconv.hip
+++ b/cabinet_amd/csrc/pwconv.hip
@@ -148,7 +148,8 @@
 bool pwconv_supported(int Ci, int Co, int P) {
     (void)P;
     return Ci % 8 == 0 && Co % 8 == 0 && Ci <= 32 * PW_MAXB && Co <= 32 * PW_MAXB &&
-           blocks_of(Ci) * blocks_of(Co) <= 8 && 32 * PW_MAXB * (Ci > Co ? Ci + 1 : Co + 1) * 4 <= 64 * 1024;
+           blocks_of(Ci) * blocks_of(Co) <= 8 && 32 * blocks_of(Co) * (Ci + 1) * 4 <= 64 * 1024 &&
+           32 * blocks_of(Ci) * (Co + 1) * 4 <= 64 * 1024;
 }
 
 static int wgrad_slabs(int B, int P) {
@@ -178,6 +179,11 @@
     return stream_launch(w, Ci, 1, Co, Ci, x, B, P, y, stream);
 }
 
+hipError_t pw_slab_sum_run(const float* slabs, int nslab, int count, float* dw, hipStream_t stream) {
+    hipLaunchKernelGGL(pw_slab_sum_kernel, dim3(ceil_div(count, 4)), dim3(256), 0, stream, slabs, nslab, count, dw);
+    return hipGetLastError();
+}
+
 template <int COB>
 static void wgrad_launch_ci(int cib, int grid, size_t lds, hipStream_t stream, const float* dy, const float* x, int Co,
                             int Ci, int P, int nchunks, int cpi, float* slabs) {
diff --git a/cabinet_amd/functional.py b/cabinet_amd/functional.py
--- a/cabinet_amd/functional.py
+++ b/cabinet_amd/functional.py
@@ -1450,6 +1450,147 @@
 
 
 
+PW_BN_BWD_ENABLED = _os.environ.get("CABINET_PW_BN_BWD", "1") != "0"
+PW_BN_BWD_GRID = 512
+PW_BN_BWD_TILE = 256
+
+_PW_BN_BWD_ROUTED = frozenset({(16, 16), (16, 64), (64, 24), (24, 72), (72, 24)})
+
+
+def pw_bn_act_supported(conv, x):
+    if not (conv.kernel_size == (1, 1) and conv.stride == (1, 1) and conv.padding == (0, 0) and conv.groups == 1
+            and conv.bias is None and conv.dilation == (1, 1) and x.is_cuda and x.dim() == 4):
+        return False
+    return bool(_lib.load().cabinet_pw_bn_bwd_supported(x.shape[0], conv.in_channels, conv.out_channels, x.shape[2] * x.shape[3]))
+
+
+def pw_bn_act_dwconv_supported(conv, x, dw):
+    return (pw_bn_act_supported(conv, x) and dwconv_supported(dw) and dw.in_channels == conv.out_channels
+            and bool(_lib.load().cabinet_pw_bn_dwconv_bwd_supported(x.shape[0], conv.in_channels, conv.out_channels, x.shape[2],
+                                                                    x.shape[3], dw.kernel_size[0], dw.stride[0])))
+
+
+def pw_bn_bwd_routed(conv, bn, x):
+    return (PW_BN_BWD_ENABLED and bn.training and torch.is_grad_enabled() and not torch.is_autocast_enabled()
+            and (conv.in_channels, conv.out_channels) in _PW_BN_BWD_ROUTED and x.dtype == torch.float32
+            and (x.requires_grad or conv.weight.requires_grad) and pw_bn_act_supported(conv, x))
+
+
+class _PwBnAct(torch.autograd.Function):
+
+    @staticmethod
+    @torch.amp.custom_fwd(device_type="cuda", cast_inputs=torch.float32)
+    def forward(fn_ctx, x, conv_w, z, bn_w, bn_b, run_mean, run_var, act, training, momentum, eps, residual):
+        lib = _lib.load()
+        x, z, bn_w, bn_b = _f32c(x), _f32c(z), _f32c(bn_w), _f32c(bn_b)
+        Co, Ci = conv_w.shape[0], conv_w.shape[1]
+        w2 = _f32c(conv_w).view(Co, Ci)
+        residual = _f32c(residual) if residual is not None else None
+        B, P = z.shape[0], z[0, 0].numel()
+        y = torch.empty_like(z)
+        mean = torch.empty(Co, dtype=torch.float32, device=z.device)
+        invstd = torch.empty(Co, dtype=torch.float32, device=z.device)
+        ws, nbytes = _workspace(lib.cabinet_bn_act_workspace_bytes(B, Co, P), z.device)
+        with torch.cuda.device(z.device):
+            rc = lib.cabinet_bn_act_fwd(_ptr(z), _ptr(bn_w), _ptr(bn_b), _ptr(run_mean), _ptr(run_var), _ptr(residual), B, Co, P,
+                                        act, int(training), float(momentum), float(eps), _ptr(y), _ptr(mean), _ptr(invstd),
+                                        _ptr(ws), nbytes, _stream_handle(z.device))
+        _lib.check(rc, "cabinet_bn_act_fwd")
+        fn_ctx.save_for_backward(x, w2, z, bn_w, bn_b, mean, invstd)
+        fn_ctx.meta = (act, bool(training), conv_w.shape)
+        return y
+
+    @staticmethod
+    @torch.amp.custom_bwd(device_type="cuda")
+    def backward(fn_ctx, g):
+        lib = _lib.load()
+        x, w2, z, bn_w, bn_b, mean, invstd = fn_ctx.saved_tensors
+        act, training, w_shape = fn_ctx.meta
+        g = _f32c(g)
+        (Co, Ci), B, P = w2.shape, x.shape[0], x.shape[2] * x.shape[3]
+        dx = torch.empty_like(x) if fn_ctx.needs_input_grad[0] else None
+        dw, dbw, dbb = torch.empty_like(w2), torch.empty_like(bn_w), torch.empty_like(bn_b)
+        ws, nbytes = _workspace(lib.cabinet_pw_bn_bwd_workspace_bytes(B, Ci, Co, P), x.device)
+        with torch.cuda.device(x.device):
+            rc = lib.cabinet_pw_bn_bwd(_ptr(g), _ptr(z), _ptr(x), _ptr(w2), _ptr(bn_w), _ptr(bn_b), _ptr(mean), _ptr(invstd), B, Ci,
+                                       Co, P, act, int(training), _ptr(dx), _ptr(dw), _ptr(dbw), _ptr(dbb), _ptr(ws), nbytes,
+                                       _stream_handle(x.device))
+        _lib.check(rc, "cabinet_pw_bn_bwd")
+        d_res = g if fn_ctx.needs_input_grad[11] else None
+        return dx, dw.view(w_shape), None, dbw, dbb, None, None, None, None, None, None, d_res
+
+
+class _PwBnActDwConv(torch.autograd.Function):
+
+    @staticmethod
+    @torch.amp.custom_fwd(device_type="cuda", cast_inputs=torch.float32)
+    def forward(fn_ctx, x, conv_w, z, bn_w, bn_b, run_mean, run_var, dw_w, act, stride, training, momentum, eps):
+        lib = _lib.load()
+        x, z, bn_w, bn_b, cw = _f32c(x), _f32c(z), _f32c(bn_w), _f32c(bn_b), _f32c(dw_w)
+        Co, Ci = conv_w.shape[0], conv_w.shape[1]
+        w2 = _f32c(conv_w).view(Co, Ci)
+        B, C, H, W = z.shape
+        K = cw.shape[-1]
+        Ho, Wo = (H + 2 * (K // 2) - K) // stride + 1, (W + 2 * (K // 2) - K) // stride + 1
+        y = torch.empty((B, C, Ho, Wo), dtype=torch.float32, device=z.device)
+        mean = torch.empty(C, dtype=torch.float32, device=z.device)
+        invstd = torch.empty(C, dtype=torch.float32, device=z.device)
+        ws, nbytes = _workspace(lib.cabinet_bn_dwconv_fwd_workspace_bytes(B, C, H, W), z.device)
+        with torch.cuda.device(z.device):
+            rc = lib.cabinet_bn_dwconv_fwd(_ptr(z), _ptr(bn_w), _ptr(bn_b), _ptr(run_mean), _ptr(run_var), _ptr(cw), B, C,
+                                           H, W, K, stride, act, int(training), float(momentum), float(eps), _ptr(y),
+                                           _ptr(mean), _ptr(invstd), _ptr(ws), nbytes, _stream_handle(z.device))
+        _lib.check(rc, "cabinet_bn_dwconv_fwd")
+        fn_ctx.save_for_backward(x, w2, z, bn_w, bn_b, cw, mean, invstd)
+        fn_ctx.meta = (act, stride, bool(training), conv_w.shape)
+        return y
+
+    @staticmethod
+    @torch.amp.custom_bwd(device_type="cuda")
+    def backward(fn_ctx, g):
+        lib = _lib.load()
+        x, w2, z, bn_w, bn_b, cw, mean, invstd = fn_ctx.saved_tensors
+        act, stride, training, w_shape = fn_ctx.meta
+        g = _f32c(g)
+        B, C, H, W = z.shape
+        Ci, K = w2.shape[1], cw.shape[-1]
+        dx = torch.empty_like(x) if fn_ctx.needs_input_grad[0] else None
+        dw, dbw, dbb, dcw = torch.empty_like(w2), torch.empty_like(bn_w), torch.empty_like(bn_b), torch.empty_like(cw)
+        ws, nbytes = _workspace(lib.cabinet_pw_bn_dwconv_bwd_workspace_bytes(B, Ci, C, H, W, K, stride), x.device)
+        with torch.cuda.device(x.device):
+            rc = lib.cabinet_pw_bn_dwconv_bwd(_ptr(g), _ptr(z), _ptr(x), _ptr(w2), _ptr(bn_w), _ptr(bn_b), _ptr(mean),
+                                              _ptr(invstd), _ptr(cw), B, Ci, C, H, W, K, stride, act, int(training), _ptr(dx),
+                                              _ptr(dw), _ptr(dbw), _ptr(dbb), _ptr(dcw), _ptr(ws), nbytes,
+                                              _stream_handle(x.device))
+        _lib.check(rc, "cabinet_pw_bn_dwconv_bwd")
+        return dx, dw.view(w_shape), None, dbw, dbb, None, None, dcw, None, None, None, None, None
+
+
+def pw_bn_act(x, conv, bn, act=None, residual=None):
+    if not x.is_cuda:
+        raise RuntimeError("pw_bn_act: device tensors only")
+    if act not in _ACT_CODES:
+        raise RuntimeError(f"pw_bn_act: unknown activation {act!r}")
+    z = pwconv(x, conv)
+    training, momentum = _bn_step(bn)
+    if residual is not None and residual.shape != z.shape:
+        raise RuntimeError(f"pw_bn_act: residual {tuple(residual.shape)} does not match {tuple(z.shape)}")
+    return _PwBnAct.apply(x, conv.weight, z.detach(), bn.weight, bn.bias, bn.running_mean, bn.running_var, _ACT_CODES[act],
+                          training, momentum, bn.eps, residual)
+
+
+def pw_bn_act_dwconv(x, conv, bn, act, dw):
+    if not x.is_cuda:
+        raise RuntimeError("pw_bn_act_dwconv: device tensors only")
+    if act not in _ACT_CODES:
+        raise RuntimeError(f"pw_bn_act_dwconv: unknown activation {act!r}")
+    z = pwconv(x, conv)
+    training, momentum = _bn_step(bn)
+    return _PwBnActDwConv.apply(x, conv.weight, z.detach(), bn.weight, bn.bias, bn.running_mean, bn.running_var, dw.weight,
+                                _ACT_CODES[act], dw.stride[0], training, momentum, bn.eps)
+
+
+
 
 PWCONV_WIDE_ENABLED = _os.environ.get("CABINET_PWCONV_WIDE", "1") != "0"
 
diff --git a/cabinet_amd/models/mobilenetv3.py b/cabinet_amd/models/mobilenetv3.py
--- a/cabinet_amd/models/mobilenetv3.py
+++ b/cabinet_amd/models/mobilenetv3.py
@@ -65,8 +65,9 @@
         if not x.is_cuda:
             y = super().forward(x)
             return y if residual is None else residual + y
-        from ..functional import (bn_act, bn_act_dwconv, dwconv, dwconv_supported, gate_act, pwconv,
-                                  pwconv_supported, pwconv_wide, pwconv_wide_supported, se_tail)
+        from ..functional import (bn_act, bn_act_dwconv, dwconv, dwconv_supported, gate_act, pw_bn_act, pw_bn_act_dwconv,
+                                  pw_bn_act_dwconv_supported, pw_bn_bwd_routed, pwconv, pwconv_supported, pwconv_wide,
+                                  pwconv_wide_supported, se_tail)
 
         layers = [m for m in self if not isinstance(m, nn.Identity)]
 
@@ -94,7 +95,19 @@
                 act = act_of(nxt)
                 x, i = gate_act(x, m.gate(x), act), i + (2 if act else 1)
             elif isinstance(m, nn.Conv2d) and m.groups == 1 and pwconv_supported(m, x):
-                x, i = pwconv(x, m), i + 1
+                nxt2 = layers[i + 2] if i + 2 < len(layers) else None
+                if (isinstance(nxt, nn.BatchNorm2d) and not isinstance(nxt2, SELayer) and pw_bn_bwd_routed(m, nxt, x)):
+                    act = act_of(nxt2)
+                    nxt3 = layers[i + 3] if act and i + 3 < len(layers) else None
+                    if isinstance(nxt3, nn.Conv2d) and nxt3.groups > 1 and pw_bn_act_dwconv_supported(m, x, nxt3):
+                        x, i = pw_bn_act_dwconv(x, m, nxt, act, nxt3), i + 4
+                    else:
+                        last = i + (3 if act else 2) >= len(layers)
+                        x, i = pw_bn_act(x, m, nxt, act, residual if last else None), i + (3 if act else 2)
+                        if last:
+                            residual = None
+                else:
+                    x, i = pwconv(x, m), i + 1
             elif isinstance(m, nn.Conv2d) and m.groups > 1 and dwconv_supported(m):
                 x, i = dwconv(x, m), i + 1
             elif pwconv_wide_supported(m, x):
diff --git a/include/cabinet_hip.h b/include/cabinet_hip.h
--- a/include/cabinet_hip.h
+++ b/include/cabinet_hip.h
@@ -265,6 +265,20 @@
 int cabinet_pwconv_bwd(const float* dy, const float* x, const float* w, int B, int Ci, int Co, int P,
                        float* dx, float* dw, void* workspace, size_t workspace_bytes, cabinet_stream_t stream);
 
+int cabinet_pw_bn_bwd_supported(int B, int Ci, int Co, int P);
+size_t cabinet_pw_bn_bwd_workspace_bytes(int B, int Ci, int Co, int P);
+int cabinet_pw_bn_bwd(const float* dy, const float* z, const float* x, const float* conv_weight, const float* bn_weight,
+                      const float* bn_bias, const float* save_mean, const float* save_invstd, int B, int Ci, int Co, int P,
+                      int act, int training, float* dx, float* dconv_weight, float* dbn_weight, float* dbn_bias,
+                      void* workspace, size_t workspace_bytes, cabinet_stream_t stream);
+int cabinet_pw_bn_dwconv_bwd_supported(int B, int Ci, int C, int H, int W, int K, int stride);
+size_t cabinet_pw_bn_dwconv_bwd_workspace_bytes(int B, int Ci, int C, int H, int W, int K, int stride);
+int cabinet_pw_bn_dwconv_bwd(const float* dy, const float* z, const float* x, const float* conv_weight,
+                             const float* bn_weight, const float* bn_bias, const float* save_mean, const float* save_invstd,
+                             const float* dw_weight, int B, int Ci, int C, int H, int W, int K, int stride, int act,
+                             int training, float* dx, float* dconv_weight, float* dbn_weight, float* dbn_bias,
+                             float* ddw_weight, void* workspace, size_t workspace_bytes, cabinet_stream_t stream);
+
 int cabinet_pwconv_wide_supported(int Ci, int Co, int P);
 size_t cabinet_pwconv_wide_wgrad_workspace_bytes(int B, int Ci, int Co, int P);
 int cabinet_pwconv_wide_wgrad(const float* dy, const float* x, int B, int Ci, int Co, int P, float* dw,
```

Measured after the change: 374.8 images/s, median of 6. 5.1% higher.
